# Benjamin-Lee/circkit

Measured on AMD Instinct MI355X. Metric: canonicalize sequences/sec (10M x 1000 b synthetic FASTA payload), higher is better.
Workload: dtype u8

## Files before the change

### circkit_amd/csrc/circkit_hip.hip

```cpp
#include <hip/hip_runtime.h>
#include <stdarg.h>
#include <stdio.h>
#include <stdlib.h>
#include <string.h>
#include <string>
#include <chrono>
#include <vector>

#include "../../include/circkit.h"
#include "canon_core.h"
#include "canon_fast.h"
#include "canon_stream.h"
#include "canon_mixed.h"
#include "fasta_host.h"
#ifndef CK_FAST_WPE
#define CK_FAST_WPE 8
#endif
#ifndef CK_STREAM_WPB
#define CK_STREAM_WPB 16
#endif
#ifndef CK_STREAM_NBUF
#define CK_STREAM_NBUF 2
#endif
#ifndef CK_FAST_BPC
#define CK_FAST_BPC 128
#endif
#include "xxh3_core.h"

namespace {

#ifndef CK_TIER_WPE
#define CK_TIER_WPE 7
#endif
template <int WPB, bool T4 = false>
__global__ __launch_bounds__(WPB * 64, CK_TIER_WPE) void canon_kernel(ck::CanonArgs a, uint32_t nvb, uint32_t* giants)
{
    extern __shared__ __attribute__((aligned(16))) uint32_t lds[];
    uint32_t* blk_count = lds + WPB * a.slice_dw;
    uint32_t* lut = blk_count + 4;
    uint32_t* lutn = lut + ck::FAST_LUT_DW;
    uint32_t live = ~0u;
    if (a.list && gridDim.x < nvb) {
        const uint32_t per = a.segs_per_block, mine = (nvb - blockIdx.x + gridDim.x - 1) / gridDim.x;
        if (threadIdx.x == 0) blk_count[1] = 0;
        __syncthreads();
        uint32_t any = 0;
        for (uint32_t t = threadIdx.x; t < mine * per; t += WPB * 64) {
            const uint32_t j = t / per, sgm = (blockIdx.x + j * gridDim.x) * per + t % per;
            if (sgm < a.in_nseg && a.list_count[sgm]) { any = 1; if (j < 32) atomicOr(blk_count + 1, 1u << j); }
        }
        if (!__syncthreads_or((int)any)) {
            if (a.defer_count)
                for (uint32_t t = threadIdx.x; t < mine; t += WPB * 64) a.defer_count[blockIdx.x + t * gridDim.x] = 0;
            return;
        }
        live = ck::uniform(blk_count[1]);
    }
    ck::fast_lut_init(lut, threadIdx.x, WPB * 64);
    ck::fast_lutn_init(lutn, threadIdx.x, WPB * 64);
    const uint32_t wib = ck::uniform(threadIdx.x >> 6);
    for (uint32_t vb = blockIdx.x, j = 0; vb < nvb; vb += gridDim.x, ++j) {
        if (j < 32 && !((live >> j) & 1u)) {
            if (threadIdx.x == 0 && a.defer_count) a.defer_count[vb] = 0;
            continue;
        }
        if (threadIdx.x == 0) *blk_count = 0;
        __syncthreads();
        ck::canon_wave_loop(a, lds + wib * a.slice_dw, lut, blk_count, vb, nvb, wib, WPB, lutn);
        __syncthreads();
        if (WPB > 1) ck::team_pass(a, lds, lut, lutn, blk_count, vb, wib, WPB, true, T4);
        if (threadIdx.x == 0 && a.defer_count) a.defer_count[vb] = *blk_count;
        if (threadIdx.x == 0 && giants && *blk_count) atomicAdd(giants, *blk_count);
    }
}

constexpr int TEAM_WAVES = 16;
__device__ __forceinline__ void team_stage_block(const ck::CanonArgs& a, uint32_t* buf, uint32_t total_dw, const uint32_t* lut, const uint32_t* lutn,
                                                 uint32_t* blk_count, uint32_t block, uint32_t wib)
{
    ck::CanonArgs solo = a;
    solo.slice_dw = total_dw;
    for (uint32_t sgm = block * a.segs_per_block; sgm < (block + 1) * a.segs_per_block && sgm < a.in_nseg; ++sgm) {
        const uint32_t count = a.list_count[sgm];
        const uint32_t* seg = a.list + (uint64_t)sgm * a.in_seg_cap;
        for (uint32_t i = 0; i < count; ++i) {
            const uint32_t entry = seg[i], rec = entry & ck::ENTRY_REC;
            const uint64_t len = a.offsets[rec + 1] - a.offsets[rec];
            bool done = false, no_2n = (entry & ck::ENTRY_NO_2N) != 0;
            if (len >= 48 && len < (1ull << 31)) {
                const uint32_t n = (uint32_t)len;
                int why = (entry & ck::ENTRY_NOT_ACGT) ? 1 : 3;
                if (why == 3 && ck::need_dw_strand2(n) <= total_dw) { why = ck::canon_record_team2(a, rec, buf, lut, blk_count + 1, wib, TEAM_WAVES); done = why == 0; }
                if (why == 1 && !(entry & ck::ENTRY_NO_2N) && ck::need_dw_2n(n) <= total_dw) {
                    done = ck::canon_record_team2n(a, rec, buf, lut, lutn, blk_count + 1, wib, TEAM_WAVES);
                    no_2n = true;
                }
                if (!done && why == 1 && ck::need_dw_strand4(n) <= total_dw) done = ck::canon_record_team4(a, rec, buf, blk_count + 1, wib, TEAM_WAVES) == 0;
            }
            if (!done) {
                if (wib == 0) {
                    bool not_acgt = (entry & ck::ENTRY_NOT_ACGT) != 0 || no_2n;
                    if (!ck::canon_record(solo, rec, buf, lut, lutn, not_acgt, no_2n)) ck::defer_record(a, blk_count, block, rec, not_acgt, no_2n);
                }
                __syncthreads();
            }
        }
    }
}
__global__ __launch_bounds__(TEAM_WAVES * 64) void canon_team_kernel(ck::CanonArgs a, uint32_t nvb, uint32_t* giants)
{
    extern __shared__ __attribute__((aligned(16))) uint32_t lds[];
    const uint32_t total_dw = TEAM_WAVES * a.slice_dw;
    uint32_t* blk_count = lds + total_dw;
    uint32_t* lut = blk_count + 4;
    uint32_t* lutn = lut + ck::FAST_LUT_DW;
    {
        const uint32_t per = a.segs_per_block, mine = blockIdx.x < nvb ? (nvb - blockIdx.x + gridDim.x - 1) / gridDim.x : 0;
        uint32_t any = 0;
        for (uint32_t t = threadIdx.x; t < mine * per; t += TEAM_WAVES * 64) {
            const uint32_t sgm = (blockIdx.x + (t / per) * gridDim.x) * per + t % per;
            if (sgm < a.in_nseg) any |= a.list_count[sgm];
        }
        if (!__syncthreads_or((int)any)) {
            for (uint32_t t = threadIdx.x; t < mine; t += TEAM_WAVES * 64) a.defer_count[blockIdx.x + t * gridDim.x] = 0;
            return;
        }
    }
    ck::fast_lut_init(lut, threadIdx.x, TEAM_WAVES * 64);
    ck::fast_lutn_init(lutn, threadIdx.x, TEAM_WAVES * 64);
    const uint32_t wib = ck::uniform(threadIdx.x >> 6);
    for (uint32_t vb = blockIdx.x; vb < nvb; vb += gridDim.x) {
        if (threadIdx.x == 0) *blk_count = 0;
        __syncthreads();
        team_stage_block(a, lds, total_dw, lut, lutn, blk_count, vb, wib);
        __syncthreads();
        if (threadIdx.x == 0) {
            a.defer_count[vb] = *blk_count;
            if (giants && *blk_count) atomicAdd(giants, *blk_count);
        }
    }
}

__global__ __launch_bounds__(TEAM_WAVES * 64) void canon_global_kernel(ck::CanonArgs a, ck::CanonArgs a2, uint32_t* scratch, uint32_t* ticket, const uint32_t* giants,
                                                                       const uint32_t* tiers_busy, uint32_t* hint_out)
{
    if (blockIdx.x == 0 && threadIdx.x == 0) *hint_out = *tiers_busy ? 2u : 1u;
    if (*giants == 0) return;
    __shared__ uint32_t blk_count[4], lut[ck::FAST_LUT_DW], lutn[ck::FAST_LUTN_DW], last;
    ck::fast_lut_init(lut, threadIdx.x, TEAM_WAVES * 64);
    ck::fast_lutn_init(lutn, threadIdx.x, TEAM_WAVES * 64);
    const uint32_t wib = ck::uniform(threadIdx.x >> 6);
    if (threadIdx.x == 0) blk_count[0] = 0;
    __syncthreads();
    team_stage_block(a, scratch + (size_t)blockIdx.x * a.slice_dw, a.slice_dw, lut, lutn, blk_count, blockIdx.x, wib);
    __syncthreads();
    if (threadIdx.x == 0) {
        a.defer_count[blockIdx.x] = blk_count[0];
        asm volatile("s_waitcnt vmcnt(0)" ::: "memory");
        __builtin_amdgcn_fence(__ATOMIC_RELEASE, "agent");
        asm volatile("s_waitcnt vmcnt(0)" ::: "memory");
        const uint32_t arrived = atomicAdd(ticket, 1u);
        last = arrived == gridDim.x - 1;
        if (last) {
            __builtin_amdgcn_fence(__ATOMIC_ACQUIRE, "agent");
            asm volatile("s_waitcnt vmcnt(0)" ::: "memory");
            *ticket = 0;
        }
    }
    __syncthreads();
    if (!last) return;
    if (threadIdx.x == 0) blk_count[0] = 0;
    __syncthreads();
    team_stage_block(a2, scratch, a2.slice_dw, lut, lutn, blk_count, 0, wib);
}

__global__ __launch_bounds__(64) void canon_global_one_kernel(ck::CanonArgs a, uint32_t* scratch)
{
    __shared__ uint32_t blk_count, lut[ck::FAST_LUT_DW], lutn[ck::FAST_LUTN_DW];
    ck::fast_lut_init(lut, threadIdx.x, 64);
    ck::fast_lutn_init(lutn, threadIdx.x, 64);
    if (threadIdx.x == 0) blk_count = 0;
    __syncthreads();
    ck::canon_wave_loop(a, scratch, lut, &blk_count, blockIdx.x, gridDim.x, 0, 1, lutn);
}

__global__ __launch_bounds__(64) void xxh3_list_kernel(const uint8_t* bytes, const uint64_t* offsets, const uint32_t* list, uint32_t count,
                                                      uint64_t* out)
{
    for (uint32_t i = blockIdx.x; i < count; i += gridDim.x) {
        const uint32_t r = list[i];
        const uint64_t off = offsets[r];
        const uint64_t h = ck::xxh3_64_wave(bytes + off, (uint32_t)(offsets[r + 1] - off));
        if (ck::lane_id() == 0) out[r] = h;
    }
}

#ifndef CK_STREAM_RPW
#define CK_STREAM_RPW 1
#endif
using StreamC = ck::StreamCfg<CK_STREAM_WPB, CK_STREAM_NBUF, CK_STREAM_RPW, 1>;
#ifndef CK_STREAM_WPB_2
#define CK_STREAM_WPB_2 8
#endif
using StreamC2 = ck::StreamCfg<CK_STREAM_WPB_2, CK_STREAM_NBUF, CK_STREAM_RPW, 2>;
#ifndef CK_STREAM_WPB_HASH
#define CK_STREAM_WPB_HASH 4
#endif
using StreamCH = ck::StreamCfg<CK_STREAM_WPB_HASH, CK_STREAM_NBUF, CK_STREAM_RPW, 1>;
#ifndef CK_STREAM_WPB_ALPHA
#define CK_STREAM_WPB_ALPHA 4
#endif
using StreamCA = ck::StreamCfg<CK_STREAM_WPB_ALPHA, CK_STREAM_NBUF, CK_STREAM_RPW, 1>;
#ifndef CK_STREAM_WPB_PAIR
#define CK_STREAM_WPB_PAIR 8
#endif
#ifndef CK_PAIR_WPE
#define CK_PAIR_WPE 6
#endif
#if CK_STREAM_WPB_PAIR
using StreamCHP = ck::StreamCfg<CK_STREAM_WPB_PAIR, CK_STREAM_NBUF, 2, 1>;
#else
using StreamCHP = StreamCH;
#endif
using StreamCAux = ck::StreamCfg<4, 4, 2, 1>;
using StreamCAux2 = ck::StreamCfg<4, 2, 2, 2>;

__host__ __device__ inline uint32_t count_shift(uint64_t n) { return n <= (1u << 17) ? 0u : (uint32_t)(63 - __builtin_clzll(n)) - 16u; }
__host__ __device__ inline uint64_t count_samples(uint64_t n) { return (n + (1ull << count_shift(n)) - 1) >> count_shift(n); }
__host__ __device__ inline uint32_t stream_mode(uint64_t two, uint64_t lng, uint64_t n)
{
    return lng && lng * 8 >= n ? 3u : (two && two * 4 >= n ? 2u : 1u);
}
constexpr uint32_t CONTENT_SAMPLES = 4096, MODE_ALPHA = 4;
constexpr uint32_t MODE_SHORT = 8, SHORT_MAX_N = 800;
__host__ __device__ inline uint32_t alpha_mode(uint64_t bad, uint64_t sampled) { return bad && bad * 16 >= sampled ? MODE_ALPHA : 0u; }
__host__ __device__ inline uint32_t batch_mode_of(uint64_t two, uint64_t lng, uint64_t n, uint64_t bad, uint64_t sampled, uint64_t shortc, bool hashed)
{
    const uint32_t m = stream_mode(two, lng, n), al = alpha_mode(bad, sampled);
    return (m == 2 && (al || hashed) ? 3u : m) | al | (m == 1 && !al && shortc * 2 >= n ? MODE_SHORT : 0u);
}
__global__ __launch_bounds__(1024) void stream_count_kernel(const uint8_t* __restrict__ bytes, const uint64_t* __restrict__ offsets, uint64_t n, uint32_t* ctl,
                                                            uint32_t* mode, uint32_t* counters, uint32_t hashed)
{
    __shared__ uint32_t blk[4];
    if (threadIdx.x < 4) blk[threadIdx.x] = 0;
    if (blockIdx.x == 0 && threadIdx.x == 3) { counters[0] = 0; counters[1] = 0; counters[3] = 0; counters[16] = 0; counters[17] = 0; }
    __syncthreads();
    const uint32_t shift = count_shift(n);
    const uint64_t ns = count_samples(n);
    uint32_t two = 0, lng = 0, sht = 0;
    for (uint64_t j = (uint64_t)blockIdx.x * 1024 + threadIdx.x; j < ns; j += (uint64_t)gridDim.x * 1024) {
        const uint64_t i = j << shift;
        const uint64_t len = offsets[i + 1] - offsets[i];
        two += len > ck::FAST_MAX_N && len <= ck::FAST2_MAX_N;
        lng += len > ck::FAST2_MAX_N;
        sht += len <= SHORT_MAX_N;
    }
    const uint64_t nc = n < CONTENT_SAMPLES ? n : CONTENT_SAMPLES, cstep = n / nc;
    uint32_t bad = 0;
    for (uint64_t k = (uint64_t)blockIdx.x * 16 + (threadIdx.x >> 6); k < nc; k += (uint64_t)gridDim.x * 16) {
        const uint64_t off = offsets[k * cstep], len = offsets[k * cstep + 1] - off;
        const uint32_t m = len < ck::FAST_MAX_N ? (uint32_t)len : ck::FAST_MAX_N, t = ck::lane_id();
        uint32_t miss = 0;
        if (m >= 16 && 16 * t < m) (void)ck::fast_pack(ck::load16(bytes + off + (16 * t + 16 <= m ? 16 * t : m - 16)), miss);
        bad += ck::ballot(miss != 0) != 0;
    }
    if (ck::ballot(two | lng) != 0) {
        const uint64_t t2 = ck::wave_sum_u64(two), tl = ck::wave_sum_u64(lng);
        if (ck::lane_id() == 0 && t2) atomicAdd(&blk[0], (uint32_t)t2);
        if (ck::lane_id() == 0 && tl) atomicAdd(&blk[1], (uint32_t)tl);
    }
    if (ck::lane_id() == 0 && bad) atomicAdd(&blk[2], bad);
    if (ck::ballot(sht != 0) != 0) {
        const uint64_t ts = ck::wave_sum_u64(sht);
        if (ck::lane_id() == 0) atomicAdd(&blk[3], (uint32_t)ts);
    }
    __syncthreads();
    if (threadIdx.x == 0) {
        if (blk[0]) atomicAdd(ctl, blk[0]);
        if (blk[1]) atomicAdd(ctl + 1, blk[1]);
        if (blk[2]) atomicAdd(ctl + 3, blk[2]);
        if (blk[3]) atomicAdd(ctl + 5, blk[3]);
        asm volatile("s_waitcnt vmcnt(0)" ::: "memory");
        if (atomicAdd(ctl + 2, 1u) == gridDim.x - 1) {
            const uint32_t t2 = atomicExch(ctl, 0u), tl = atomicExch(ctl + 1, 0u), tb = atomicExch(ctl + 3, 0u), ts = atomicExch(ctl + 5, 0u);
            *mode = batch_mode_of(t2, tl, ns, tb, nc, ts, hashed != 0);
            atomicExch(ctl + 2, 0u);
        }
    }
}
__device__ __forceinline__ uint32_t batch_mode(const uint32_t* __restrict__ mode, uint32_t host_mode)
{
    return host_mode ? host_mode & 15u : *mode;
}
template <bool HASH, bool AUX, bool ALPHA>
__global__ __launch_bounds__(256) void canon_rescue_kernel(ck::CanonArgs a, const uint32_t* __restrict__ mode_word, uint32_t host_mode, uint32_t* mode_out,
                                                           uint32_t* tiers_busy)
{
    const uint32_t mode = batch_mode(mode_word, host_mode);
    if (!AUX && ((mode & MODE_ALPHA) != 0) != ALPHA) return;
    if (!AUX && (mode & 3) == 3) return;
    if (blockIdx.x == 0 && threadIdx.x == 0) *mode_out = (host_mode >> 31) ? *mode_word : mode;
    const bool all_records = (mode & 3) == 3;
    if (!all_records) {
        const uint32_t mine = blockIdx.x < a.in_nseg ? (a.in_nseg - blockIdx.x + gridDim.x - 1) / gridDim.x : 0;
        uint32_t any = 0;
        for (uint32_t t = threadIdx.x; t < mine; t += 256) any |= a.list_count[blockIdx.x + t * gridDim.x];
        if (!__syncthreads_or((int)any)) {
            for (uint32_t t = threadIdx.x; t < mine; t += 256) a.defer_count[blockIdx.x + t * gridDim.x] = 0;
            return;
        }
    }
    __shared__ uint32_t lut[ck::FAST_LUT_DW], seg_count;
    ck::fast_lut_init(lut, threadIdx.x, 256);
    ck::RescueState<HASH, AUX> st;
    if (HASH) st.hc = ck::fast_hash_const();
    const uint32_t wib = ck::uniform(threadIdx.x >> 6);
    uint32_t passed_on = 0, walked = 0;
    for (uint32_t sgm = blockIdx.x; sgm < a.in_nseg; sgm += gridDim.x) {
        if (threadIdx.x == 0) seg_count = 0;
        __syncthreads();
        ck::canon_rescue_segment<HASH, AUX, ALPHA>(a, lut, st, &seg_count, sgm, wib, 4, all_records);
        __syncthreads();
        if (threadIdx.x == 0) { a.defer_count[sgm] = seg_count; passed_on += seg_count; ++walked; }
    }
    if (threadIdx.x == 0 && passed_on > walked) *tiers_busy = 1;
}

#ifdef CK_MIXED_TIMELINE
__device__ uint64_t g_timeline[3 * 65536];
#endif
#ifndef CK_MIXED_WPB_PURE
#define CK_MIXED_WPB_PURE 8
#endif
#ifndef CK_MIXED_WPB_HASH
#define CK_MIXED_WPB_HASH 2
#endif
#ifndef CK_MIXED_WPB_N
#define CK_MIXED_WPB_N 4
#endif
constexpr int mixed_wpb(bool nm, bool hash) { return nm ? CK_MIXED_WPB_N : (hash ? CK_MIXED_WPB_HASH : CK_MIXED_WPB_PURE); }
template <bool NM, bool HASH>
__device__ __forceinline__ void canon_mixed_body(const ck::CanonArgs& a, const uint32_t* __restrict__ mode_word, uint32_t host_mode, uint32_t* mode_out, uint32_t* tiers_busy,
                                                 uint32_t* ticket)
{
    constexpr int WPB = mixed_wpb(NM, HASH);
    const uint32_t mode = batch_mode(mode_word, host_mode);
    if ((mode & 3) != 3 || ((mode & MODE_ALPHA) != 0) != NM) return;
    if (blockIdx.x == 0 && threadIdx.x == 0) *mode_out = (host_mode >> 31) ? *mode_word : mode;
#ifdef CK_MIXED_TIMELINE
    const uint64_t tl_start = wall_clock64();
#endif
    extern __shared__ __attribute__((aligned(16))) uint32_t lds[];
    uint32_t* blk_count = lds + WPB * a.slice_dw;
    uint32_t* lut = blk_count + 4;
    uint32_t* lutn = lut + ck::FAST_LUT_DW;
    uint32_t* htab = lutn + ck::LEAN_LUTN_DW;
    ck::fast_lut_init(lut, threadIdx.x, 64 * WPB);
    if (NM) ck::lean_lutn_init(lutn, threadIdx.x, 64 * WPB);
    if (HASH) ck::lean_hash_table_init(htab, threadIdx.x);
    ck::RescueState<HASH, false> st;
    if (HASH) {
        st.hc.k0 = ck::xsec64(8 * (ck::lane_id() >> 2) + 16 * (ck::lane_id() & 3));
        st.hc.k1 = ck::xsec64(8 * (ck::lane_id() >> 2) + 16 * (ck::lane_id() & 3) + 8);
    }
    const uint32_t wib = ck::uniform(threadIdx.x >> 6);
    uint32_t* slice = lds + wib * a.slice_dw;
    const uint64_t payload_end = a.offsets[a.n_records];
    uint32_t passed_on = 0, walked = 0, static_sgm = blockIdx.x;
    for (;;) {
        if (threadIdx.x == 0) { blk_count[0] = 0; blk_count[1] = ticket ? atomicAdd(ticket, 1u) : static_sgm; }
        static_sgm += gridDim.x;
        __syncthreads();
        const uint32_t sgm = blk_count[1];
        if (sgm >= a.in_nseg) break;
        ck::canon_mixed_segment<NM, HASH>(a, slice, lut, st, blk_count, sgm, wib, WPB, payload_end, htab, lutn);
        __syncthreads();
        if (threadIdx.x == 0) { a.defer_count[sgm] = *blk_count; passed_on += *blk_count; ++walked; }
    }
    if (threadIdx.x == 0) {
        if (passed_on > walked) *tiers_busy = 1;
        if (ticket && atomicAdd(ticket + 1, 1u) == gridDim.x - 1) { atomicExch(ticket, 0u); atomicExch(ticket + 1, 0u); }
    }
#ifdef CK_MIXED_TIMELINE
    if (threadIdx.x == 0 && blockIdx.x < 65536) {
        uint32_t hwid;
        asm volatile("s_getreg_b32 %0, hwreg(HW_REG_HW_ID)" : "=s"(hwid));
        uint32_t xcc;
        asm volatile("s_getreg_b32 %0, hwreg(HW_REG_XCC_ID)" : "=s"(xcc));
        g_timeline[3 * blockIdx.x] = tl_start; g_timeline[3 * blockIdx.x + 1] = wall_clock64();
        g_timeline[3 * blockIdx.x + 2] = ((uint64_t)xcc << 32) | hwid;
    }
#endif
}
#ifndef CK_MIXED_NM_VGPR
#define CK_MIXED_NM_VGPR 48
#endif
#ifndef CK_MIXED_H_VGPR
#define CK_MIXED_H_VGPR 40
#endif
#ifndef CK_MIXED_N_SLICE
#define CK_MIXED_N_SLICE 1904
#endif
#ifdef CK_MIXED_WAVES
#define CK_MIXED_ATTR(VGPR, NM, HASH) __launch_bounds__(64 * mixed_wpb(NM, HASH), CK_MIXED_WAVES)
#else
#define CK_MIXED_ATTR(VGPR, NM, HASH) __launch_bounds__(64 * mixed_wpb(NM, HASH)) __attribute__((amdgpu_num_vgpr(VGPR)))
#endif
#define CK_MIXED_KERNEL(NAME, NM, HASH, VGPR)                                                                                                  \
    __global__ CK_MIXED_ATTR(VGPR, NM, HASH) void NAME(ck::CanonArgs a, const uint32_t* __restrict__ mode_word,   \
                                                                                     uint32_t host_mode, uint32_t* mode_out, uint32_t* tiers_busy, uint32_t* ticket) \
    {                                                                                                                                          \
        canon_mixed_body<NM, HASH>(a, mode_word, host_mode, mode_out, tiers_busy, ticket);                                                     \
    }
CK_MIXED_KERNEL(canon_mixed_kernel, false, false, 36)
CK_MIXED_KERNEL(canon_mixed_n_kernel, true, false, CK_MIXED_NM_VGPR)
CK_MIXED_KERNEL(canon_mixed_h_kernel, false, true, CK_MIXED_H_VGPR)
CK_MIXED_KERNEL(canon_mixed_nh_kernel, true, true, CK_MIXED_NM_VGPR)
#undef CK_MIXED_KERNEL

#ifndef CK_GROUP_HASH
#define CK_GROUP_HASH 1
#endif
template <class StreamC, bool HASH, bool AUX, bool PERSIST, bool ALPHA = false>
__global__ __launch_bounds__(StreamC::WPB * 64, (HASH && !AUX && StreamC::ROWS == 1 && (ALPHA || StreamC::RPW == 2)) ? CK_PAIR_WPE : (StreamC::WPB >= 8 || (ALPHA && !HASH && !AUX)) ? CK_FAST_WPE : 4) void canon_stream_kernel(ck::CanonArgs a, const uint32_t* __restrict__ mode,
                                                                                                             uint32_t host_mode, uint32_t nvb)
{
    const uint32_t bm = batch_mode(mode, host_mode);
    if ((bm & 3) != (uint32_t)StreamC::ROWS) return;
    constexpr bool HAS_ALPHA_TWIN = StreamC::ROWS == 1 && !AUX;
    if (HAS_ALPHA_TWIN && ((bm & MODE_ALPHA) != 0) != ALPHA) return;
    if (HAS_ALPHA_TWIN && !ALPHA && !HASH && ((bm & MODE_SHORT) != 0) != (StreamC::RPW == 2)) return;
    constexpr bool GH = CK_GROUP_HASH && HASH && !AUX && StreamC::ROWS == 1 && (StreamC::RPW == 1 || !ALPHA) && StreamC::GROUP <= 16;
    constexpr bool PAIR = GH && StreamC::RPW == 2;
    constexpr bool PAIR_B = !HASH && !AUX && !ALPHA && StreamC::ROWS == 1 && StreamC::RPW == 2;
    __shared__ __attribute__((aligned(16))) uint32_t lds[StreamC::LDS_DW + (GH ? ck::gh_lds_dw<(int)StreamC::GROUP, PAIR>() : PAIR_B ? StreamC::GROUP * ck::PAIR_SCRATCH_DW : 0)];
    uint32_t* lut = lds + StreamC::NBUF * StreamC::BUF_DW;
    uint32_t* blk_count = lut + ck::FAST_LUT_DW;
    uint32_t* gh = lds + StreamC::LDS_DW;
    ck::fast_lut_init(lut, threadIdx.x, StreamC::WPB * 64);
    if (GH) ck::group_hash_init(gh + 2 * StreamC::GROUP * ck::GH_STRIDE_DW, threadIdx.x);
    if (PAIR) ck::group_hash_secret_init(gh + 2 * StreamC::GROUP * ck::GH_STRIDE_DW + ck::GH_CONST_DW, threadIdx.x);
    if (!PERSIST) {
        if (threadIdx.x == 0) *blk_count = 0;
        __syncthreads();
        ck::canon_stream_wave_loop<StreamC, HASH, AUX, GH, ALPHA>(a, lut, lds, blk_count, blockIdx.x, gridDim.x, gh);
        __syncthreads();
        if (threadIdx.x == 0) a.defer_count[blockIdx.x] = *blk_count;
        return;
    }
    for (uint32_t vb = blockIdx.x; vb < nvb; vb += gridDim.x) {
        if (threadIdx.x == 0) *blk_count = 0;
        __syncthreads();
        ck::canon_stream_wave_loop<StreamC, HASH, AUX, GH, ALPHA>(a, lut, lds, blk_count, vb, nvb, gh);
        ck::vmem_wait<0>();
        __syncthreads();
        if (threadIdx.x == 0) a.defer_count[vb] = *blk_count;
    }
}

__global__ __launch_bounds__(256) void xxh3_kernel(const uint8_t* bytes, const uint64_t* offsets, uint64_t n_records,
                                                   uint64_t* out, const uint8_t* hashed, const uint32_t* view, const uint8_t* comp)
{
    const uint32_t wave = ck::uniform(blockIdx.x * 4 + (threadIdx.x >> 6));
    const uint32_t n_waves = gridDim.x * 4;
    const ck::XWaveConst xk = ck::xwave_const();
    __shared__ uint8_t comp_lds[256];
    if (view) { comp_lds[threadIdx.x] = comp[threadIdx.x]; __syncthreads(); comp = comp_lds; }
    if (!hashed) {
        for (uint64_t r = wave; r < n_records; r += n_waves) {
            const uint64_t off = offsets[r];
            const uint64_t h = ck::xxh3_64_wave(bytes + off, (uint32_t)(offsets[r + 1] - off), xk);
            if (ck::lane_id() == 0) out[r] = h;
        }
        return;
    }
    const uint64_t per_wave = (n_records + n_waves - 1) / n_waves;
    const uint32_t span = per_wave >= 512 ? 512u : (per_wave <= 64 ? 64u : (uint32_t)((per_wave + 63) / 64) * 64u);
    for (uint64_t big = (uint64_t)wave * span; big < n_records; big += (uint64_t)n_waves * span) {
      const uint64_t f0 = big + 8 * ck::lane_id();
      uint64_t flags8 = ~0ull;
      if (f0 < n_records && 8 * ck::lane_id() < span) {
          flags8 = *reinterpret_cast<const uint64_t*>(hashed + f0);
          if (n_records - f0 < 8) flags8 |= ~0ull << (8 * (n_records - f0));
      }
      if (ck::ballot(((flags8 - 0x0101010101010101ull) & ~flags8 & 0x8080808080808080ull) != 0) == 0) continue;
      for (uint64_t base = big; base < big + span && base < n_records; base += 64) {
        const uint64_t mine = base + ck::lane_id();
        const bool need = mine < n_records && !hashed[mine];
        uint64_t todo = ck::ballot(need);
        if (!todo) continue;
        const uint64_t my_off = need ? offsets[mine] : 0;
        const uint32_t my_len = need ? (uint32_t)(offsets[mine + 1] - my_off) : 0u;
        const bool mine_short = need && my_len <= 240u;
        const uint64_t shorts = ck::ballot(mine_short);
        if (shorts) {
            if (mine_short) {
                const uint8_t* p = bytes + my_off;
                uint64_t h;
                if (view) {
                    const uint32_t v = view[mine], rot = v & 0x7FFFFFFFu;
                    h = ck::xxh3_short(ck::XView{ p, my_len, rot < my_len ? rot : 0u, (v >> 31) != 0, comp }, my_len);
                } else h = ck::xxh3_short(ck::XPlain{ p }, my_len);
                out[mine] = h;
            }
            todo &= ~shorts;
        }
        while (todo) {
            const uint32_t l = (uint32_t)ck::ffs64(todo);
            todo &= todo - 1;
            const uint64_t off = ((uint64_t)ck::readlane((uint32_t)(my_off >> 32), l) << 32) | ck::readlane((uint32_t)my_off, l);
            const uint32_t len = ck::readlane(my_len, l);
            const uint64_t h = view ? ck::xxh3_64_wave_view(bytes + off, len, view[base + l], comp, xk) : ck::xxh3_64_wave(bytes + off, len, xk);
            if (ck::lane_id() == 0) out[base + l] = h;
        }
      }
    }
}

__device__ __forceinline__ uint64_t splitmix64(uint64_t x)
{
    x += 0x9E3779B97F4A7C15ULL;
    x = (x ^ (x >> 30)) * 0xBF58476D1CE4E5B9ULL;
    x = (x ^ (x >> 27)) * 0x94D049BB133111EBULL;
    return x ^ (x >> 31);
}

__global__ __launch_bounds__(256) void synth_fill_kernel(uint64_t seed, uint64_t first_base, uint64_t n_bases,
                                                         uint8_t* out)
{
    const uint64_t key = seed * 0xD1342543DE82EF95ULL;
    const uint64_t stride = (uint64_t)gridDim.x * blockDim.x * 16;
    for (uint64_t i = ((uint64_t)blockIdx.x * blockDim.x + threadIdx.x) * 16; i < n_bases; i += stride) {
        const uint64_t g0 = first_base + i;
        uint64_t wi = g0 >> 5, w = splitmix64(key + wi);
        uint32_t o[4] = { 0, 0, 0, 0 };
#pragma unroll
        for (int b = 0; b < 16; ++b) {
            const uint64_t g = g0 + b;
            if ((g >> 5) != wi) { wi = g >> 5; w = splitmix64(key + wi); }
            const uint32_t code = (uint32_t)(w >> (2 * (g & 31))) & 3u;
            o[b >> 2] |= ((0x54474341u >> (8 * code)) & 0xFFu) << (8 * (b & 3));
        }
        if (i + 16 <= n_bases) {
            ck::store16(out + i, ck::u32x4{ o[0], o[1], o[2], o[3] });
        } else {
            for (uint64_t b = 0; i + b < n_bases; ++b) out[i + b] = (uint8_t)(o[b >> 2] >> (8 * (b & 3)));
        }
    }
}

typedef uint32_t copy_v4 __attribute__((ext_vector_type(4)));
template <int UNROLL>
__global__ __launch_bounds__(256) void bench_copy_kernel(const copy_v4* __restrict__ in, copy_v4* __restrict__ out, uint64_t n16)
{
    const uint64_t stride = (uint64_t)gridDim.x * 256 * UNROLL;
    uint64_t i = (uint64_t)blockIdx.x * 256 * UNROLL + threadIdx.x;
    for (; i + 256 * (UNROLL - 1) < n16; i += stride) {
        copy_v4 r[UNROLL];
#pragma unroll
        for (int u = 0; u < UNROLL; ++u) r[u] = in[i + u * 256];
#pragma unroll
        for (int u = 0; u < UNROLL; ++u) out[i + u * 256] = r[u];
    }
    for (; i < n16; i += 256) out[i] = in[i];
}

__global__ void fixed_offsets_kernel(uint64_t base, uint64_t len, uint64_t n, uint64_t* off)
{
    const uint64_t stride = (uint64_t)gridDim.x * blockDim.x;
    for (uint64_t i = (uint64_t)blockIdx.x * blockDim.x + threadIdx.x; i <= n; i += stride) off[i] = base + i * len;
}

constexpr uint64_t UNIQ_EMPTY = ~0ull;
struct __attribute__((aligned(16))) UniqSlot { unsigned long long key, val; };
__device__ __forceinline__ uint64_t uniq_slot(uint64_t h, uint64_t mask) { return (h ^ (h >> 29)) & mask; }
__device__ __forceinline__ UniqSlot uniq_peek(const UniqSlot* p)
{
    typedef unsigned long long v2 __attribute__((ext_vector_type(2)));
    const v2 v = *reinterpret_cast<const v2*>(p);
    return UniqSlot{ v.x, v.y };
}
__device__ __forceinline__ bool uniq_fold(UniqSlot* t, uint64_t mask, uint64_t h, unsigned long long v)
{
    if (h == UNIQ_EMPTY) { atomicMin(&t[mask + 1].val, v); return true; }
    uint64_t s = uniq_slot(h, mask), probes = 0;
    for (;;) {
        const UniqSlot cur = uniq_peek(t + s);
        if (cur.key == h) {
            if (cur.val > v) atomicMin(&t[s].val, v);
            return true;
        }
        if (cur.key == UNIQ_EMPTY) {
            const unsigned long long old = atomicCAS(&t[s].key, (unsigned long long)UNIQ_EMPTY, (unsigned long long)h);
            if (old == UNIQ_EMPTY || old == h) { atomicMin(&t[s].val, v); return true; }
        }
        s = (s + 1) & mask;
        if (++probes > mask) return false;
    }
}

__global__ __launch_bounds__(256) void uniq_insert_kernel(const uint64_t* __restrict__ hash, const uint64_t* __restrict__ index, uint64_t n, uint64_t base,
                                                          UniqSlot* t, uint64_t mask, uint32_t* status)
{
    const uint64_t stride = (uint64_t)gridDim.x * blockDim.x;
    for (uint64_t i = (uint64_t)blockIdx.x * blockDim.x + threadIdx.x; i < n; i += stride)
        if (!uniq_fold(t, mask, hash[i], index ? index[i] : base + i)) atomicAdd(status, 1u);
}

__global__ __launch_bounds__(256) void uniq_lookup_kernel(const uint64_t* __restrict__ hash, uint64_t n, const UniqSlot* __restrict__ t, uint64_t mask,
                                                          uint64_t* first_seen, uint8_t* keep, uint64_t base)
{
    const uint64_t stride = (uint64_t)gridDim.x * blockDim.x;
    for (uint64_t i = (uint64_t)blockIdx.x * blockDim.x + threadIdx.x; i < n; i += stride) {
        const uint64_t h = hash[i];
        uint64_t r = UNIQ_EMPTY;
        if (h == UNIQ_EMPTY) {
            r = t[mask + 1].val;
        } else {
            uint64_t s = uniq_slot(h, mask), probes = 0;
            for (;;) {
                const UniqSlot cur = uniq_peek(t + s);
                if (cur.key == h) { r = cur.val; break; }
                if (cur.key == UNIQ_EMPTY || ++probes > mask) break;
                s = (s + 1) & mask;
            }
        }
        first_seen[i] = r;
        if (keep) keep[i] = r == base + i;
    }
}

__device__ __forceinline__ bool uniq_fold_local(UniqSlot* t, uint64_t mask, uint64_t h, uint32_t i)
{
    if (h == UNIQ_EMPTY) { atomicMin(reinterpret_cast<unsigned int*>(&t[mask + 1].val), i); return true; }
    uint64_t s = uniq_slot(h, mask), probes = 0;
    for (;;) {
        const UniqSlot cur = uniq_peek(t + s);
        unsigned int* halves = reinterpret_cast<unsigned int*>(&t[s].val);
        if (cur.key == h) {
            const uint32_t lo = (uint32_t)cur.val, hi = (uint32_t)(cur.val >> 32);
            if ((lo < hi ? lo : hi) > i) atomicMin(halves, i);
            return true;
        }
        if (cur.key == UNIQ_EMPTY) {
            const unsigned long long old = atomicCAS(&t[s].key, (unsigned long long)UNIQ_EMPTY, (unsigned long long)h);
            if (old == UNIQ_EMPTY) { halves[1] = i; return true; }
            if (old == h) { atomicMin(halves, i); return true; }
        }
        s = (s + 1) & mask;
        if (++probes > mask) return false;
    }
}
__global__ __launch_bounds__(256) void uniq_resolve_insert_kernel(const uint64_t* __restrict__ hash, uint64_t n, UniqSlot* t, uint64_t mask, uint32_t* status,
                                                                  const uint32_t* only_if = nullptr)
{
    if (only_if && *only_if == 0) return;
    const uint64_t stride = (uint64_t)gridDim.x * blockDim.x;
    for (uint64_t i = (uint64_t)blockIdx.x * blockDim.x + threadIdx.x; i < n; i += stride)
        if (!uniq_fold_local(t, mask, hash[i], (uint32_t)i)) atomicAdd(status, 1u);
}
__global__ __launch_bounds__(256) void uniq_resolve_lookup_kernel(const uint64_t* __restrict__ hash, uint64_t n, const UniqSlot* __restrict__ t, uint64_t mask,
                                                                  uint64_t* first_seen, uint8_t* keep, uint64_t base, const uint32_t* only_if = nullptr)
{
    if (only_if && *only_if == 0) return;
    const uint64_t stride = (uint64_t)gridDim.x * blockDim.x;
    for (uint64_t i = (uint64_t)blockIdx.x * blockDim.x + threadIdx.x; i < n; i += stride) {
        const uint64_t h = hash[i];
        uint64_t v = UNIQ_EMPTY;
        if (h == UNIQ_EMPTY) {
            v = t[mask + 1].val;
        } else {
            uint64_t s = uniq_slot(h, mask), probes = 0;
            for (;;) {
                const UniqSlot cur = uniq_peek(t + s);
                if (cur.key == h) { v = cur.val; break; }
                if (cur.key == UNIQ_EMPTY || ++probes > mask) break;
                s = (s + 1) & mask;
            }
        }
        const uint32_t lo = (uint32_t)v, hi = (uint32_t)(v >> 32), r = lo < hi ? lo : hi;
        first_seen[i] = r == 0xFFFFFFFFu ? UNIQ_EMPTY : base + r;
        if (keep) keep[i] = r == (uint32_t)i;
    }
}

__global__ __launch_bounds__(256) void uniq_rehash_kernel(const UniqSlot* __restrict__ old, uint64_t oslots, UniqSlot* t, uint64_t mask)
{
    const uint64_t stride = (uint64_t)gridDim.x * blockDim.x;
    for (uint64_t i = (uint64_t)blockIdx.x * blockDim.x + threadIdx.x; i < oslots; i += stride) {
        const UniqSlot e = uniq_peek(old + i);
        if (i + 1 == oslots) { if (e.val != UNIQ_EMPTY) atomicMin(&t[mask + 1].val, e.val); continue; }
        if (e.key != UNIQ_EMPTY) (void)uniq_fold(t, mask, e.key, e.val);
    }
}

constexpr uint32_t UNIQ_MAX_WORLD = 64;
__device__ __forceinline__ uint32_t uniq_owner(uint64_t h, uint32_t world) { return (uint32_t)((h >> 20) & 0x7FFFFFFFu) % world; }
__global__ __launch_bounds__(256) void uniq_partition_count_kernel(const uint64_t* __restrict__ hash, uint64_t n, uint32_t world, unsigned long long* counts)
{
    __shared__ uint32_t hist[UNIQ_MAX_WORLD];
    if (threadIdx.x < UNIQ_MAX_WORLD) hist[threadIdx.x] = 0;
    __syncthreads();
    const uint64_t stride = (uint64_t)gridDim.x * blockDim.x;
    for (uint64_t i = (uint64_t)blockIdx.x * blockDim.x + threadIdx.x; i < n; i += stride) atomicAdd(&hist[uniq_owner(hash[i], world)], 1u);
    __syncthreads();
    if (threadIdx.x < world && hist[threadIdx.x]) atomicAdd(&counts[threadIdx.x], (unsigned long long)hist[threadIdx.x]);
}
__global__ __launch_bounds__(256) void uniq_partition_scatter_kernel(const uint64_t* __restrict__ hash, uint64_t n, uint64_t base, uint32_t world,
                                                                     const unsigned long long* __restrict__ counts, unsigned long long* cursor,
                                                                     uint64_t* rows, uint32_t* slot)
{
    __shared__ uint32_t hist[UNIQ_MAX_WORLD];
    __shared__ unsigned long long first[UNIQ_MAX_WORLD], start[UNIQ_MAX_WORLD];
    constexpr uint32_t PER = 4;
    const uint64_t chunk = 256ull * PER;
    if (threadIdx.x < UNIQ_MAX_WORLD) {
        unsigned long long v = threadIdx.x < world ? counts[threadIdx.x] : 0ull, incl = v;
        for (uint32_t d = 1; d < UNIQ_MAX_WORLD; d <<= 1) {
            const uint32_t lo = ck::shfl((uint32_t)incl, threadIdx.x - d), hi = ck::shfl((uint32_t)(incl >> 32), threadIdx.x - d);
            if (threadIdx.x >= d) incl += ((unsigned long long)hi << 32) | lo;
        }
        first[threadIdx.x] = incl - v;
    }
    for (uint64_t c0 = (uint64_t)blockIdx.x * chunk; c0 < n; c0 += (uint64_t)gridDim.x * chunk) {
        if (threadIdx.x < UNIQ_MAX_WORLD) hist[threadIdx.x] = 0;
        __syncthreads();
        uint32_t rank[PER];
#pragma unroll
        for (uint32_t k = 0; k < PER; ++k) {
            const uint64_t i = c0 + k * 256 + threadIdx.x;
            rank[k] = i < n ? atomicAdd(&hist[uniq_owner(hash[i], world)], 1u) : 0u;
        }
        __syncthreads();
        if (threadIdx.x < world)
            start[threadIdx.x] = first[threadIdx.x] + (hist[threadIdx.x] ? atomicAdd(&cursor[threadIdx.x], (unsigned long long)hist[threadIdx.x]) : 0ull);
        __syncthreads();
#pragma unroll
        for (uint32_t k = 0; k < PER; ++k) {
            const uint64_t i = c0 + k * 256 + threadIdx.x;
            if (i < n) {
                const uint64_t h = hash[i];
                const uint64_t pos = start[uniq_owner(h, world)] + rank[k];
                typedef unsigned long long v2 __attribute__((ext_vector_type(2)));
                *reinterpret_cast<v2*>(rows + 2 * pos) = v2{ h, base + i };
                slot[i] = (uint32_t)pos;
            }
        }
        __syncthreads();
    }
}
__global__ __launch_bounds__(256) void uniq_insert_rows_kernel(const uint64_t* __restrict__ rows, uint64_t n, UniqSlot* t, uint64_t mask, uint32_t* status)
{
    const uint64_t stride = (uint64_t)gridDim.x * blockDim.x;
    for (uint64_t i = (uint64_t)blockIdx.x * blockDim.x + threadIdx.x; i < n; i += stride) {
        const UniqSlot r = uniq_peek(reinterpret_cast<const UniqSlot*>(rows) + i);
        if (!uniq_fold(t, mask, r.key, r.val)) atomicAdd(status, 1u);
    }
}
__global__ __launch_bounds__(256) void uniq_lookup_rows_kernel(const uint64_t* __restrict__ rows, uint64_t n, const UniqSlot* __restrict__ t, uint64_t mask,
                                                               uint64_t* answers)
{
    const uint64_t stride = (uint64_t)gridDim.x * blockDim.x;
    for (uint64_t i = (uint64_t)blockIdx.x * blockDim.x + threadIdx.x; i < n; i += stride) {
        const uint64_t h = rows[2 * i];
        uint64_t r = UNIQ_EMPTY;
        if (h == UNIQ_EMPTY) {
            r = t[mask + 1].val;
        } else {
            uint64_t s = uniq_slot(h, mask), probes = 0;
            for (;;) {
                const UniqSlot cur = uniq_peek(t + s);
                if (cur.key == h) { r = cur.val; break; }
                if (cur.key == UNIQ_EMPTY || ++probes > mask) break;
                s = (s + 1) & mask;
            }
        }
        answers[i] = r;
    }
}
__global__ __launch_bounds__(256) void uniq_gather_kernel(const uint64_t* __restrict__ answers, const uint32_t* __restrict__ slot, uint64_t n, uint64_t base,
                                                          uint64_t* first_seen, uint8_t* keep)
{
    const uint64_t stride = (uint64_t)gridDim.x * blockDim.x;
    for (uint64_t i = (uint64_t)blockIdx.x * blockDim.x + threadIdx.x; i < n; i += stride) {
        const uint64_t r = answers[slot[i]];
        first_seen[i] = r;
        if (keep) keep[i] = r == base + i;
    }
}

__global__ __launch_bounds__(256) void uniq_clear_kernel(UniqSlot* t, uint64_t slots, uint32_t* overflow, const uint32_t* only_if = nullptr)
{
    if (only_if && *only_if == 0) return;
    typedef unsigned long long v2 __attribute__((ext_vector_type(2)));
    if (overflow && blockIdx.x == 0 && threadIdx.x == 0) *overflow = 0;
    const uint64_t stride = (uint64_t)gridDim.x * blockDim.x;
    for (uint64_t i = (uint64_t)blockIdx.x * blockDim.x + threadIdx.x; i < slots; i += stride)
        *reinterpret_cast<v2*>(t + i) = v2{ UNIQ_EMPTY, UNIQ_EMPTY };
}

#ifndef CK_BKT_NW
#define CK_BKT_NW 512
#endif
constexpr uint32_t BKT_NW = CK_BKT_NW, BKT_SLOTS = 4096, BKT_MAX = 3072, BKT_KEYS = 2600, BKT_MAX_LOG2 = 13;
__device__ __forceinline__ uint32_t bkt_of(uint64_t h, uint32_t log2b) { return (uint32_t)(h >> (64 - log2b)); }
__global__ __launch_bounds__(1024) void uniq_bkt_count_kernel(const uint64_t* __restrict__ hash, uint64_t n, uint64_t per, uint32_t log2b, uint32_t* counts,
                                                              uint32_t* flag, uint32_t* overflow)
{
    extern __shared__ uint32_t bkt_lds[];
    const uint32_t B = 1u << log2b;
    for (uint32_t b = threadIdx.x; b < B; b += 1024) bkt_lds[b] = 0;
    if (blockIdx.x == 0 && threadIdx.x == 0) { *flag = 0; *overflow = 0; }
    __syncthreads();
    const uint64_t i0 = (uint64_t)blockIdx.x * per, i1 = i0 + per < n ? i0 + per : n;
    for (uint64_t i = i0 + threadIdx.x; i < i1; i += 1024) atomicAdd(&bkt_lds[bkt_of(hash[i], log2b)], 1u);
    __syncthreads();
    for (uint32_t b = threadIdx.x; b < B; b += 1024) counts[(uint64_t)blockIdx.x * B + b] = bkt_lds[b];
}
__global__ __launch_bounds__(1024) void uniq_bkt_colscan_kernel(uint32_t* counts, uint32_t B, uint32_t* tot)
{
    __shared__ uint32_t seg[16][64];
    constexpr uint32_t PER = BKT_NW / 16;
    const uint32_t bl = threadIdx.x & 63, sg = threadIdx.x >> 6, b = blockIdx.x * 64 + bl;
    uint32_t sum = 0;
    for (uint32_t w = sg * PER; w < (sg + 1) * PER; ++w) sum += counts[(uint64_t)w * B + b];
    seg[sg][bl] = sum;
    __syncthreads();
    uint32_t run = 0;
    for (uint32_t k = 0; k < sg; ++k) run += seg[k][bl];
    for (uint32_t w = sg * PER; w < (sg + 1) * PER; ++w) {
        const uint64_t k = (uint64_t)w * B + b;
        const uint32_t cnt = counts[k];
        counts[k] = run;
        run += cnt;
    }
    if (sg == 15) tot[b] = run;
}
__global__ __launch_bounds__(1024) void uniq_bkt_basescan_kernel(const uint32_t* __restrict__ tot, uint32_t B, uint32_t* base)
{
    __shared__ uint32_t part[1024];
    const uint32_t items = (B + 1023) / 1024, b0 = threadIdx.x * items;
    uint32_t sum = 0;
    for (uint32_t k = 0; k < items; ++k) if (b0 + k < B) sum += tot[b0 + k];
    part[threadIdx.x] = sum;
    __syncthreads();
    for (uint32_t d = 1; d < 1024; d <<= 1) {
        const uint32_t v = threadIdx.x >= d ? part[threadIdx.x - d] : 0u;
        __syncthreads();
        part[threadIdx.x] += v;
        __syncthreads();
    }
    uint32_t run = part[threadIdx.x] - sum;
    for (uint32_t k = 0; k < items; ++k) if (b0 + k < B) { base[b0 + k] = run; run += tot[b0 + k]; }
    if (threadIdx.x == 1023) base[B] = part[1023];
}
__global__ __launch_bounds__(1024) void uniq_bkt_scatter_kernel(const uint64_t* __restrict__ hash, uint64_t n, uint64_t per, uint32_t log2b,
                                                                const uint32_t* __restrict__ counts, const uint32_t* __restrict__ base, uint64_t* rows,
                                                                uint64_t* first_seen, uint64_t base_index)
{
    extern __shared__ uint32_t bkt_lds[];
    const uint32_t B = 1u << log2b;
    for (uint32_t b = threadIdx.x; b < B; b += 1024) bkt_lds[b] = base[b] + counts[(uint64_t)blockIdx.x * B + b];
    __syncthreads();
    const uint64_t i0 = (uint64_t)blockIdx.x * per, i1 = i0 + per < n ? i0 + per : n;
    typedef unsigned long long v2 __attribute__((ext_vector_type(2)));
    constexpr int U = 4;
    uint64_t i = i0 + threadIdx.x;
    for (; i + (U - 1) * 1024 < i1; i += U * 1024) {
        uint64_t h[U];
#pragma unroll
        for (int u = 0; u < U; ++u) h[u] = hash[i + u * 1024];
#pragma unroll
        for (int u = 0; u < U; ++u) {
            const uint32_t pos = atomicAdd(&bkt_lds[bkt_of(h[u], log2b)], 1u);
            *reinterpret_cast<v2*>(rows + 2 * (uint64_t)pos) = v2{ h[u], i + u * 1024 };
            first_seen[i + u * 1024] = base_index + i + u * 1024;
        }
    }
    for (; i < i1; i += 1024) {
        const uint64_t h = hash[i];
        const uint32_t pos = atomicAdd(&bkt_lds[bkt_of(h, log2b)], 1u);
        *reinterpret_cast<v2*>(rows + 2 * (uint64_t)pos) = v2{ h, i };
        first_seen[i] = base_index + i;
    }
}
#ifndef BKT_RESOLVE_T
#define BKT_RESOLVE_T 1024
#endif
__global__ __launch_bounds__(BKT_RESOLVE_T) void uniq_bkt_resolve_kernel(const uint64_t* __restrict__ rows, const uint32_t* __restrict__ base, uint64_t base_index,
                                                               uint64_t* first_seen, uint8_t* keep, uint32_t* flag)
{
    __shared__ unsigned long long keys[BKT_SLOTS];
    __shared__ uint32_t idx[BKT_SLOTS], special;
    const uint32_t r0 = base[blockIdx.x], cnt = base[blockIdx.x + 1] - r0;
    if (cnt == 0) return;
    if (cnt > BKT_MAX) { if (threadIdx.x == 0) atomicExch(flag, 1u); return; }
    for (uint32_t s = threadIdx.x; s < BKT_SLOTS; s += BKT_RESOLVE_T) { keys[s] = UNIQ_EMPTY; idx[s] = 0xFFFFFFFFu; }
    if (threadIdx.x == 0) special = 0xFFFFFFFFu;
    __syncthreads();
    constexpr uint32_t RPT = (BKT_MAX + BKT_RESOLVE_T - 1) / BKT_RESOLVE_T;
    uint64_t hk[RPT];
    uint32_t ik[RPT];
#pragma unroll
    for (uint32_t k = 0; k < RPT; ++k) {
        const uint32_t r = threadIdx.x + k * BKT_RESOLVE_T;
        hk[k] = 0; ik[k] = 0xFFFFFFFFu;
        if (r < cnt) { const UniqSlot row = uniq_peek(reinterpret_cast<const UniqSlot*>(rows) + r0 + r); hk[k] = row.key; ik[k] = (uint32_t)row.val; }
    }
#pragma unroll
    for (uint32_t k = 0; k < RPT; ++k) {
        if (ik[k] == 0xFFFFFFFFu) continue;
        const uint64_t h = hk[k];
        if (h == UNIQ_EMPTY) { atomicMin(&special, ik[k]); continue; }
        uint32_t s = (uint32_t)(h ^ (h >> 29)) & (BKT_SLOTS - 1);
        for (;;) {
            const unsigned long long old = atomicCAS(&keys[s], (unsigned long long)UNIQ_EMPTY, (unsigned long long)h);
            if (old == UNIQ_EMPTY || old == h) { atomicMin(&idx[s], ik[k]); break; }
            s = (s + 1) & (BKT_SLOTS - 1);
        }
    }
    __syncthreads();
#pragma unroll
    for (uint32_t k = 0; k < RPT; ++k) {
        if (ik[k] == 0xFFFFFFFFu) continue;
        const uint64_t h = hk[k];
        uint32_t m;
        if (h == UNIQ_EMPTY) m = special;
        else {
            uint32_t s = (uint32_t)(h ^ (h >> 29)) & (BKT_SLOTS - 1);
            while (keys[s] != h) s = (s + 1) & (BKT_SLOTS - 1);
            m = idx[s];
        }
        if (m != ik[k]) first_seen[ik[k]] = base_index + m;
    }
}
__global__ __launch_bounds__(256) void uniq_keep_kernel(const uint64_t* __restrict__ first_seen, uint64_t n, uint64_t base, uint8_t* keep, const uint32_t* skip_if)
{
    if (skip_if && *skip_if != 0) return;
    const uint64_t stride = (uint64_t)gridDim.x * blockDim.x;
    for (uint64_t i = (uint64_t)blockIdx.x * blockDim.x + threadIdx.x; i < n; i += stride) keep[i] = first_seen[i] == base + i;
}

#ifndef CK_RESCUE_BPC
#define CK_RESCUE_BPC 8
#endif
#ifndef CK_TIER_BPC
#define CK_TIER_BPC 128
#endif
#ifndef CK_TIER_BPC_IDLE
#define CK_TIER_BPC_IDLE 8
#endif
#ifndef CK_TIER_A
#define CK_TIER_A 1280
#endif
#ifndef CK_TIER_B1
#define CK_TIER_B1 1900
#endif
#ifndef CK_TIER_B2
#define CK_TIER_B2 3324
#endif
constexpr int N_TIERS = 5;
constexpr uint32_t TIER_DW[N_TIERS] = { CK_TIER_A, CK_TIER_B1, CK_TIER_B2, 9980, CK_LUT_STRIDE == 1 ? 40188u : 31996u };
constexpr uint32_t TIER_EXTRA_DW = 4 + ck::FAST_LUT_DW + ck::FAST_LUTN_DW;
constexpr uint32_t TIER_D_DW = TIER_DW[N_TIERS - 1];
constexpr int BATCH_TIERS = 3;
constexpr uint32_t BATCH_SLICE_DW[BATCH_TIERS - 1] = { CK_TIER_A, 9980 / 4 };
constexpr uint32_t TEAM_SLICE_DW = TIER_D_DW / 16;
constexpr int N_CU = 256;

}

struct circkit_ctx {
    int device = -1;
    hipStream_t own_stream = nullptr, stream = nullptr;
    hipEvent_t ev0 = nullptr, ev1 = nullptr;
    hipEvent_t ev_order = nullptr;
    static constexpr int MAX_PARTS = 32;
    hipStream_t s_in = nullptr, s_out = nullptr;
    hipEvent_t ev_in[MAX_PARTS] = {}, ev_done[MAX_PARTS] = {}, ev_head = nullptr;
    bool timed = false;
    std::string err;
    uint8_t* d_comp = nullptr;
    uint32_t* d_counters = nullptr;
    uint32_t* d_lists[N_TIERS + 1] = {};
    uint32_t* d_seg_counts = nullptr;
    uint64_t list_cap = 0, seg_alloc = 0;
    uint8_t *d_in = nullptr, *d_out = nullptr, *d_strand = nullptr;
    uint64_t* d_off = nullptr; uint32_t* d_idx = nullptr; uint64_t* d_hash = nullptr;
    uint64_t cap_bytes = 0, cap_rec = 0;
    uint32_t* d_view = nullptr; uint64_t cap_view = 0;
    uint8_t* d_hashed = nullptr; uint64_t cap_hashed = 0;
    uint32_t* d_gscratch = nullptr; uint64_t cap_gscratch = 0;
    uint64_t gscratch_default = 256ull << 20;
    uint64_t* h_off = nullptr;
    uint64_t h_off_cap = 0;
    volatile uint32_t* h_mode = nullptr;
    uint32_t* d_mode = nullptr;
    UniqSlot* d_table = nullptr;
    uint64_t uniq_mask = 0, uniq_count = 0;
    uint32_t mode_seen = 0;
    bool uniq_local = false;
    bool uniq_lost = false;

    void* orfs = nullptr;
    void (*orfs_release)(void*) = nullptr;
    void* monomerize = nullptr;
    void (*monomerize_release)(void*) = nullptr;
};

hipStream_t ck_ctx_stream(circkit_ctx* c) { return c->stream; }
int ck_ctx_device(circkit_ctx* c) { return c->device; }
int ck_ctx_fail(circkit_ctx* c, int code, const char* msg) { c->err = msg; return code; }
void** ck_ctx_orfs_slot(circkit_ctx* c, void (*release)(void*)) { c->orfs_release = release; return &c->orfs; }
void** ck_ctx_monomerize_slot(circkit_ctx* c, void (*release)(void*)) { c->monomerize_release = release; return &c->monomerize; }

namespace {

int fail(circkit_ctx* c, int code, const char* fmt, ...)
{
    char buf[512];
    va_list ap; va_start(ap, fmt); vsnprintf(buf, sizeof buf, fmt, ap); va_end(ap);
    if (c) c->err = buf;
    return code;
}

#define CK_HIP(c, call)                                                                             \
    do {                                                                                            \
        hipError_t e_ = (call);                                                                     \
        if (e_ != hipSuccess)                                                                       \
            return fail(c, e_ == hipErrorOutOfMemory ? CIRCKIT_ERR_OOM : CIRCKIT_ERR_HIP,           \
                        "%s failed: %s", #call, hipGetErrorString(e_));                             \
    } while (0)

int ensure_lists(circkit_ctx* c, uint64_t entries, uint64_t segs)
{
    if (entries > c->list_cap) {
        c->list_cap = 0;
        for (int i = 0; i < N_TIERS + 1; ++i) {
            if (c->d_lists[i]) { (void)hipFree(c->d_lists[i]); c->d_lists[i] = nullptr; }
            CK_HIP(c, hipMalloc(&c->d_lists[i], entries * sizeof(uint32_t)));
        }
        c->list_cap = entries;
    }
    if (segs > c->seg_alloc) {
        if (c->d_seg_counts) { (void)hipFree(c->d_seg_counts); c->d_seg_counts = nullptr; }
        c->seg_alloc = 0;
        CK_HIP(c, hipMalloc(&c->d_seg_counts, (N_TIERS + 1) * segs * sizeof(uint32_t)));
        c->seg_alloc = segs;
    }
    return CIRCKIT_OK;
}

int ensure_gscratch(circkit_ctx* c, uint64_t bytes)
{
    if (bytes <= c->cap_gscratch) return CIRCKIT_OK;
    if (c->d_gscratch) { (void)hipFree(c->d_gscratch); c->d_gscratch = nullptr; c->cap_gscratch = 0; }
    CK_HIP(c, hipMalloc(&c->d_gscratch, bytes));
    c->cap_gscratch = bytes;
    return CIRCKIT_OK;
}

inline uint64_t worst_case_dw(uint64_t n) { return 2 * ((n + 3) / 4 + 2) + (n + 31) / 32 + 1 + 64; }
constexpr uint64_t GSLICE1_DW = 1ull << 20;

int launch_canon(circkit_ctx* c, const uint8_t* d_bytes, const uint64_t* d_offsets, uint64_t n, uint8_t* d_out,
                 uint32_t* d_idx, uint8_t* d_strand, uint64_t* d_hash, uint32_t flags, uint32_t host_mode = 0, bool keep_status = false)
{
#ifdef CK_FORCE_HOST_MODE
    if (!host_mode) host_mode = CK_FORCE_HOST_MODE;
#endif
    if (n >= (1ull << 30)) return fail(c, CIRCKIT_ERR_INVALID_ARG, "n_records must be < 2^30");
    CK_HIP(c, hipSetDevice(c->device));
    if (n == 0) { c->timed = false; return CIRCKIT_OK; }
    const bool device_decides = host_mode == 0;
    uint32_t guess_flag = 0;
    if (device_decides) {
        static const bool no_guess = getenv("CIRCKIT_NO_MODE_GUESS") != nullptr;
        const uint32_t seen = *c->h_mode & 15u;
        if (!no_guess && (seen & 3u) && seen == c->mode_seen) { host_mode = seen; guess_flag = 0x80000000u; }
        c->mode_seen = seen;
        static const bool dbg = getenv("CIRCKIT_DEBUG_MODE_GUESS") != nullptr;
        if (dbg) fprintf(stderr, "[mode guess] n=%llu report=%u -> %s\n", (unsigned long long)n, seen, guess_flag ? "guessed" : "decided on the device");
    }
    const uint32_t kmode = host_mode | guess_flag;
    const bool aux = d_idx || d_strand || (flags & ck::CK_FLAG_FWD_ONLY);
    const uint64_t per_step = aux ? StreamCAux::GROUP : StreamC::GROUP;
    const uint64_t blocks = (n + per_step - 1) / per_step;
    unsigned G = (unsigned)(blocks < (uint64_t)N_CU * CK_FAST_BPC ? blocks : (uint64_t)N_CU * CK_FAST_BPC);
    const unsigned G_small = (unsigned)(n < (uint64_t)N_CU * 16 ? n : (uint64_t)N_CU * 16);
    if (G < G_small) G = G_small;
    uint32_t cap = (uint32_t)(per_step * ((blocks + G - 1) / G));
    uint32_t all_cap = (uint32_t)((n + G - 1) / G);
    uint32_t taper_seg0 = 0, taper_log2 = 0;
#ifndef CK_NO_TAPER
#ifndef CK_TAPER_DIV
#define CK_TAPER_DIV 16
#endif
    if (G >= 4096 && all_cap >= (2u << CK_TAPER_GENS)) {
        while ((2u << taper_log2) <= G / CK_TAPER_DIV) ++taper_log2;
        const uint64_t gen = 1ull << taper_log2;
        taper_seg0 = G - (uint32_t)(CK_TAPER_GENS * gen);
        auto tapered = [&](uint32_t A) { uint64_t t = 0; for (int j = 1; j <= CK_TAPER_GENS; ++j) t += A >> j; return t; };
        while ((uint64_t)taper_seg0 * all_cap + gen * tapered(all_cap) < n) ++all_cap;
        if (cap < all_cap) cap = all_cap;
    }
#endif
    int rc = ensure_lists(c, (uint64_t)G * cap + 1024ull * cap, G < 256u ? 256u : G);
    if (rc) return rc;
    if (!c->d_gscratch && (rc = ensure_gscratch(c, c->gscratch_default))) return rc;
    uint32_t* view = nullptr;
    if (d_hash && !d_out) {
        if (n > c->cap_view) {
            if (c->d_view) { (void)hipFree(c->d_view); c->d_view = nullptr; c->cap_view = 0; }
            CK_HIP(c, hipMalloc(&c->d_view, (n + n / 8 + 64) * sizeof(uint32_t)));
            c->cap_view = n + n / 8 + 64;
        }
        view = c->d_view;
    }
    if (d_hash) {
        if (n > c->cap_hashed) {
            if (c->d_hashed) { (void)hipFree(c->d_hashed); c->d_hashed = nullptr; c->cap_hashed = 0; }
            CK_HIP(c, hipMalloc(&c->d_hashed, n + n / 8 + 64));
            c->cap_hashed = n + n / 8 + 64;
        }
        CK_HIP(c, hipMemsetAsync(c->d_hashed, 0, n, c->stream));
    }
    if (!device_decides) CK_HIP(c, hipMemsetAsync(c->d_counters, 0, (keep_status ? 3 : 4) * sizeof(uint32_t), c->stream));
    CK_HIP(c, hipEventRecord(c->ev0, c->stream));
    ck::CanonArgs a{};
    a.bytes = d_bytes; a.offsets = d_offsets; a.n_records = n;
    a.out_bytes = d_out; a.out_index = d_idx; a.out_strand = d_strand; a.out_hash = d_hash; a.hashed = c->d_hashed; a.out_view = view;
    a.comp_lut = c->d_comp; a.status = c->d_counters + 3; a.flags = flags;
    a.list = nullptr; a.list_count = nullptr; a.all_seg_cap = all_cap; a.taper_seg0 = taper_seg0; a.taper_log2 = taper_log2;
    a.defer_list = c->d_lists[0]; a.defer_count = c->d_seg_counts; a.out_seg_cap = cap;
    a.slice_dw = 0;
    const uint32_t* counts = c->d_counters + 5;
    {
        if (device_decides) {
            const uint64_t ns = count_samples(n);
            const unsigned cgrid = (unsigned)((ns + 1023) / 1024 < 128 ? (ns + 1023) / 1024 : 128);
            hipLaunchKernelGGL(stream_count_kernel, dim3(cgrid), dim3(1024), 0, c->stream, d_bytes, d_offsets, n, c->d_counters + 8, c->d_counters + 5, c->d_counters, (d_hash && !aux) ? 1u : 0u);
        }
        const uint32_t seen = *c->h_mode;
        const uint32_t expect = host_mode ? host_mode & 3 : ((seen & 3) ? seen & 3 : 1u);
        const unsigned small = G < 2u * N_CU ? G : 2u * N_CU;
        const dim3 block(StreamC::WPB * 64), block_aux(StreamCAux::WPB * 64), block_h(StreamCH::WPB * 64), block_hp(StreamCHP::WPB * 64), block_a(StreamCA::WPB * 64), block_2(StreamC2::WPB * 64);
        const uint32_t expect_alpha = host_mode ? host_mode & MODE_ALPHA : seen & MODE_ALPHA;
        for (uint32_t rows = 1; rows <= 2; ++rows) {
            if (host_mode && (host_mode & 3) != rows) continue;
            for (uint32_t alpha = 0; alpha <= (rows == 1 && !aux ? 1u : 0u); ++alpha) {
                if (host_mode && rows == 1 && !aux && ((host_mode & MODE_ALPHA) != 0) != (alpha != 0)) continue;
                const bool full = expect == rows && (rows != 1 || aux || (expect_alpha != 0) == (alpha != 0));
                const dim3 grid(full ? G : small);
#define CK_LAUNCH_STREAM(CFG, H, A, BLK, AL)                                                                                         \
                do {                                                                                                                \
                    if (full) hipLaunchKernelGGL((canon_stream_kernel<CFG, H, A, false, AL>), grid, BLK, 0, c->stream, a, counts, kmode, G); \
                    else hipLaunchKernelGGL((canon_stream_kernel<CFG, H, A, true, AL>), grid, BLK, 0, c->stream, a, counts, kmode, G);       \
                } while (0)
                if (rows == 1) {
                    if (aux) CK_LAUNCH_STREAM(StreamCAux, true, true, block_aux, false);
                    else if (d_hash) { if (alpha) CK_LAUNCH_STREAM(StreamCH, true, false, block_h, true); else CK_LAUNCH_STREAM(StreamCHP, true, false, block_hp, false); }
                    else if (alpha) CK_LAUNCH_STREAM(StreamCA, false, false, block_a, true);
                    else {
                        const bool expect_short = ((host_mode ? host_mode : seen) & MODE_SHORT) != 0;
                        for (int sh = 0; sh < 2; ++sh) {
                            if (host_mode && (sh != 0) != expect_short) continue;
                            const bool full_sh = full && (sh != 0) == expect_short;
                            const dim3 grid_sh(full_sh ? G : small);
                            if (sh) { if (full_sh) hipLaunchKernelGGL((canon_stream_kernel<StreamCHP, false, false, false, false>), grid_sh, block_hp, 0, c->stream, a, counts, kmode, G);
                                      else hipLaunchKernelGGL((canon_stream_kernel<StreamCHP, false, false, true, false>), grid_sh, block_hp, 0, c->stream, a, counts, kmode, G); }
                            else { if (full_sh) hipLaunchKernelGGL((canon_stream_kernel<StreamC, false, false, false, false>), grid_sh, block, 0, c->stream, a, counts, kmode, G);
                                   else hipLaunchKernelGGL((canon_stream_kernel<StreamC, false, false, true, false>), grid_sh, block, 0, c->stream, a, counts, kmode, G); }
                        }
                    }
                } else {
                    if (aux) CK_LAUNCH_STREAM(StreamCAux2, true, true, block_aux, false);
                    else if (d_hash) CK_LAUNCH_STREAM(StreamC2, true, false, block_2, false);
                    else CK_LAUNCH_STREAM(StreamC2, false, false, block_2, false);
                }
#undef CK_LAUNCH_STREAM
            }
        }
    }
    unsigned nseg = G;
    uint32_t seg_cap = cap;
    {
        const unsigned grid = nseg < (unsigned)N_CU * CK_RESCUE_BPC ? nseg : (unsigned)N_CU * CK_RESCUE_BPC;
        a.list = c->d_lists[0]; a.list_count = c->d_seg_counts;
        a.in_nseg = nseg; a.in_seg_cap = seg_cap; a.segs_per_block = 1;
        a.defer_list = c->d_lists[1]; a.defer_count = c->d_seg_counts + c->seg_alloc; a.out_seg_cap = seg_cap;
#ifdef CK_NO_PINNED_MODE
        uint32_t* mode_out = c->d_counters + 6;
#else
        uint32_t* mode_out = c->d_mode;
#endif
        const bool mixed_has_it = host_mode && !aux && (host_mode & 3) == 3;
        const bool lean = (!host_mode || !(host_mode & MODE_ALPHA)) && !mixed_has_it, alpha = (!host_mode || (host_mode & MODE_ALPHA)) && !mixed_has_it;
        if (aux) hipLaunchKernelGGL((canon_rescue_kernel<true, true, false>), dim3(grid), dim3(256), 0, c->stream, a, counts, kmode, mode_out, c->d_counters + 1);
        else if (d_hash) {
            if (lean) hipLaunchKernelGGL((canon_rescue_kernel<true, false, false>), dim3(grid), dim3(256), 0, c->stream, a, counts, kmode, mode_out, c->d_counters + 1);
            if (alpha) hipLaunchKernelGGL((canon_rescue_kernel<true, false, true>), dim3(grid), dim3(256), 0, c->stream, a, counts, kmode, mode_out, c->d_counters + 1);
        } else {
            if (lean) hipLaunchKernelGGL((canon_rescue_kernel<false, false, false>), dim3(grid), dim3(256), 0, c->stream, a, counts, kmode, mode_out, c->d_counters + 1);
            if (alpha) hipLaunchKernelGGL((canon_rescue_kernel<false, false, true>), dim3(grid), dim3(256), 0, c->stream, a, counts, kmode, mode_out, c->d_counters + 1);
        }
    }
    if (!aux && (!host_mode || (host_mode & 3) == 3)) {
        const uint32_t seen = *c->h_mode;
        const unsigned walking = nseg < (unsigned)N_CU * CK_RESCUE_BPC ? nseg : (unsigned)N_CU * CK_RESCUE_BPC;
#ifdef CK_NO_PINNED_MODE
        uint32_t* mode_out = c->d_counters + 6;
#else
        uint32_t* mode_out = c->d_mode;
#endif
        for (uint32_t nm = 0; nm < 2; ++nm) {
            if (host_mode && ((host_mode & MODE_ALPHA) != 0) != (nm != 0)) continue;
            const bool expected = host_mode ? true : ((seen & 3) == 3 && ((seen & MODE_ALPHA) != 0) == (nm != 0));
            const unsigned resident = (unsigned)N_CU * (20u / (unsigned)mixed_wpb(true, false));
#ifdef CK_MIXED_N_STATIC
            const unsigned full = nseg;
#else
            const unsigned full = nm ? (nseg < resident ? nseg : resident) : nseg;
#endif
            const unsigned grid = expected ? full : walking;
#ifdef CK_MIXED_N_STATIC
            uint32_t* ticket = nullptr;
#else
            uint32_t* ticket = nm ? c->d_counters + 16 : nullptr;
#endif
            a.slice_dw = nm ? CK_MIXED_N_SLICE : TIER_DW[0];
            const int mwpb = nm ? mixed_wpb(true, d_hash != nullptr) : (d_hash ? mixed_wpb(false, true) : mixed_wpb(false, false));
            const size_t shmem = ((size_t)mwpb * a.slice_dw + 4 + ck::FAST_LUT_DW + ck::LEAN_LUTN_DW + (d_hash ? ck::LEAN_HASH_TABLE_DW : 0)) * 4;
            if (d_hash) {
                if (nm) hipLaunchKernelGGL(canon_mixed_nh_kernel, dim3(grid), dim3(64 * mwpb), shmem, c->stream, a, counts, kmode, mode_out, c->d_counters + 1, ticket);
                else hipLaunchKernelGGL(canon_mixed_h_kernel, dim3(grid), dim3(64 * mwpb), shmem, c->stream, a, counts, kmode, mode_out, c->d_counters + 1, ticket);
            } else {
                if (nm) hipLaunchKernelGGL(canon_mixed_n_kernel, dim3(grid), dim3(64 * mwpb), shmem, c->stream, a, counts, kmode, mode_out, c->d_counters + 1, ticket);
                else hipLaunchKernelGGL(canon_mixed_kernel, dim3(grid), dim3(64 * mwpb), shmem, c->stream, a, counts, kmode, mode_out, c->d_counters + 1, ticket);
            }
        }
    }
#ifdef CK_DEBUG_DUMP
    {
        (void)hipStreamSynchronize(c->stream);
        std::vector<uint32_t> cnt(nseg);
        (void)hipMemcpy(cnt.data(), c->d_seg_counts + c->seg_alloc, nseg * 4, hipMemcpyDeviceToHost);
        uint64_t total = 0; unsigned shown = 0;
        if (getenv("CK_DUMP_HIST")) {
            std::vector<uint32_t> ents((size_t)nseg * seg_cap);
            (void)hipMemcpy(ents.data(), c->d_lists[1], ents.size() * 4, hipMemcpyDeviceToHost);
            std::vector<uint64_t> offs(n + 1);
            (void)hipMemcpy(offs.data(), d_offsets, (n + 1) * 8, hipMemcpyDeviceToHost);
            uint64_t hist[2][32] = {}, bytes[2] = {};
            for (unsigned sg = 0; sg < nseg; ++sg)
                for (uint32_t k = 0; k < cnt[sg]; ++k) {
                    const uint32_t e = ents[(size_t)sg * seg_cap + k]; const uint64_t len = offs[(e & ck::ENTRY_REC) + 1] - offs[e & ck::ENTRY_REC];
                    hist[e >> 31][63 - __builtin_clzll(len | 1)]++; bytes[e >> 31] += len;
                }
            for (int f = 0; f < 2; ++f) { fprintf(stderr, "[dump] flag %d (%llu bytes):", f, (unsigned long long)bytes[f]); for (int b = 0; b < 32; ++b) if (hist[f][b]) fprintf(stderr, " 2^%d:%llu", b, (unsigned long long)hist[f][b]); fprintf(stderr, "\n"); }
        }
        for (unsigned sg = 0; sg < nseg; ++sg) {
            total += cnt[sg];
            for (uint32_t k = 0; k < cnt[sg] && shown < 12; ++k, ++shown) {
                uint32_t e = 0; uint64_t o[2];
                (void)hipMemcpy(&e, c->d_lists[1] + (uint64_t)sg * seg_cap + k, 4, hipMemcpyDeviceToHost);
                (void)hipMemcpy(o, d_offsets + (e & ck::ENTRY_REC), 16, hipMemcpyDeviceToHost);
                fprintf(stderr, "[dump] seg %u entry %u: rec %u flag %u len %llu\n", sg, k, e & ck::ENTRY_REC, e >> 31, (unsigned long long)(o[1] - o[0]));
            }
        }
        fprintf(stderr, "[dump] stage A input: %llu records in %u segments\n", (unsigned long long)total, nseg);
    }
#endif
    const bool tiers_idle = c->h_mode[1] == 1;
    for (int t = 0; t < BATCH_TIERS; ++t) {
        const bool last = t == BATCH_TIERS - 1;
        const unsigned spb = t == 0 ? 1 : (last ? (nseg + N_CU - 1) / N_CU : (nseg >= 16u * N_CU ? 4 : 1));
        const unsigned grid = (nseg + spb - 1) / spb;
        a.list = c->d_lists[t + 1]; a.list_count = c->d_seg_counts + (uint64_t)(t + 1) * c->seg_alloc;
        a.in_nseg = nseg; a.in_seg_cap = seg_cap; a.segs_per_block = spb;
        a.defer_list = last ? c->d_lists[0] : c->d_lists[t + 2];
        a.defer_count = last ? c->d_seg_counts : c->d_seg_counts + (uint64_t)(t + 2) * c->seg_alloc;
        a.out_seg_cap = spb * seg_cap;
        a.slice_dw = last ? TEAM_SLICE_DW : BATCH_SLICE_DW[t];
        const unsigned bpc = tiers_idle ? CK_TIER_BPC_IDLE : CK_TIER_BPC;
        const unsigned launched = grid < (unsigned)N_CU * bpc ? grid : (unsigned)N_CU * bpc;
        if (last) hipLaunchKernelGGL(canon_team_kernel, dim3(launched), dim3(TEAM_WAVES * 64), (TEAM_WAVES * TEAM_SLICE_DW + TIER_EXTRA_DW) * 4, c->stream, a, grid, c->d_counters);
        else if (tiers_idle) hipLaunchKernelGGL((canon_kernel<4, false>), dim3(launched), dim3(256), (4 * a.slice_dw + TIER_EXTRA_DW) * 4, c->stream, a, grid, (uint32_t*)nullptr);
        else hipLaunchKernelGGL((canon_kernel<4, true>), dim3(launched), dim3(256), (4 * a.slice_dw + TIER_EXTRA_DW) * 4, c->stream, a, grid, (uint32_t*)nullptr);
        nseg = grid;
        seg_cap = spb * seg_cap;
    }
    {
        const uint64_t cap_dw = c->cap_gscratch / 4;
        const uint64_t slice1 = cap_dw < GSLICE1_DW ? cap_dw : GSLICE1_DW;
        const unsigned max_w1 = (unsigned)(cap_dw / slice1 < 64 ? cap_dw / slice1 : 64);
        const unsigned spb1 = (nseg + max_w1 - 1) / max_w1, w1 = (nseg + spb1 - 1) / spb1;
        a.list = c->d_lists[0]; a.list_count = c->d_seg_counts;
        a.in_nseg = nseg; a.in_seg_cap = seg_cap; a.segs_per_block = spb1;
        a.defer_list = c->d_lists[1]; a.defer_count = c->d_seg_counts + c->seg_alloc; a.out_seg_cap = spb1 * seg_cap;
        a.slice_dw = (uint32_t)slice1;
        ck::CanonArgs a2 = a;
        a2.list = c->d_lists[1]; a2.list_count = c->d_seg_counts + c->seg_alloc;
        a2.in_nseg = w1; a2.in_seg_cap = spb1 * seg_cap; a2.segs_per_block = w1;
        a2.defer_list = nullptr; a2.defer_count = nullptr; a2.out_seg_cap = 0;
        a2.slice_dw = (uint32_t)(cap_dw < 0xFFFFFFFFull ? cap_dw : 0xFFFFFFFFull);
        hipLaunchKernelGGL(canon_global_kernel, dim3(w1), dim3(TEAM_WAVES * 64), 0, c->stream, a, a2, c->d_gscratch, c->d_counters + 2, (const uint32_t*)c->d_counters,
                           (const uint32_t*)(c->d_counters + 1), c->d_mode + 1);
    }
    if (d_hash) {
        if (view) hipLaunchKernelGGL(xxh3_kernel, dim3(G < 2048u ? G : 2048u), dim3(256), 0, c->stream, d_bytes, d_offsets, n, d_hash, (const uint8_t*)c->d_hashed,
                                     (const uint32_t*)view, (const uint8_t*)c->d_comp);
        else hipLaunchKernelGGL(xxh3_kernel, dim3(G < 2048u ? G : 2048u), dim3(256), 0, c->stream, d_out, d_offsets, n, d_hash, (const uint8_t*)c->d_hashed,
                                (const uint32_t*)nullptr, (const uint8_t*)nullptr);
    }
    CK_HIP(c, hipEventRecord(c->ev1, c->stream));
    CK_HIP(c, hipGetLastError());
    c->timed = true;
    return CIRCKIT_OK;
}

int launch_single(circkit_ctx* c, const uint8_t* d_bytes, const uint64_t* d_offsets, uint64_t len, uint8_t* d_out, uint32_t* d_idx,
                  uint8_t* d_strand, uint64_t* d_hash, uint32_t flags)
{
    ck::CanonArgs a{};
    a.bytes = d_bytes; a.offsets = d_offsets; a.n_records = 1;
    a.out_bytes = d_out; a.out_index = d_idx; a.out_strand = d_strand; a.out_hash = nullptr; a.hashed = nullptr;
    a.comp_lut = c->d_comp; a.status = c->d_counters + 3; a.flags = flags;
    CK_HIP(c, hipMemsetAsync(c->d_counters + 3, 0, sizeof(uint32_t), c->stream));
    const uint64_t need = worst_case_dw(len);
    int t = 0;
    while (t < N_TIERS && TIER_DW[t] < need) ++t;
    if (t < N_TIERS) {
        a.slice_dw = TIER_DW[t];
        hipLaunchKernelGGL(canon_kernel<1>, dim3(1), dim3(64), (TIER_DW[t] + TIER_EXTRA_DW) * 4, c->stream, a, 1u, (uint32_t*)nullptr);
    } else {
        int rc = ensure_gscratch(c, need * 4);
        if (rc) return rc;
        a.slice_dw = (uint32_t)(need < 0xFFFFFFFFull ? need : 0xFFFFFFFFull);
        hipLaunchKernelGGL(canon_global_one_kernel, dim3(1), dim3(64), 0, c->stream, a, c->d_gscratch);
    }
    if (d_hash) hipLaunchKernelGGL(xxh3_kernel, dim3(1), dim3(256), 0, c->stream, d_out, d_offsets, (uint64_t)1, d_hash, (const uint8_t*)nullptr, (const uint32_t*)nullptr, (const uint8_t*)nullptr);
    CK_HIP(c, hipGetLastError());
    c->timed = false;
    return CIRCKIT_OK;
}

template <class T>
int grow(circkit_ctx* c, T*& p, uint64_t want_elems)
{
    if (p) { (void)hipFree(p); p = nullptr; }
    CK_HIP(c, hipMalloc(&p, want_elems * sizeof(T)));
    return CIRCKIT_OK;
}

int ensure_staging(circkit_ctx* c, uint64_t bytes, uint64_t recs)
{
    if (bytes + 64 > c->cap_bytes) {
        const uint64_t nb = bytes + bytes / 8 + 4096;
        c->cap_bytes = 0;
        int rc;
        if ((rc = grow(c, c->d_in, nb))) return rc;
        if ((rc = grow(c, c->d_out, nb))) return rc;
        c->cap_bytes = nb;
    }
    if (recs + 1 > c->cap_rec) {
        const uint64_t nr = recs + recs / 8 + 1024;
        c->cap_rec = 0;
        int rc;
        if ((rc = grow(c, c->d_off, nr))) return rc;
        if ((rc = grow(c, c->d_idx, nr))) return rc;
        if ((rc = grow(c, c->d_strand, nr))) return rc;
        if ((rc = grow(c, c->d_hash, nr))) return rc;
        c->cap_rec = nr;
    }
    return CIRCKIT_OK;
}

int host_batch_enqueue(circkit_ctx* c, const uint8_t* bytes, const uint64_t* offsets, uint64_t n, uint8_t* out,
                       uint32_t* idx, uint8_t* strand, uint64_t* hash, uint32_t flags);
int host_batch(circkit_ctx* c, const uint8_t* bytes, const uint64_t* offsets, uint64_t n, uint8_t* out,
               uint32_t* idx, uint8_t* strand, uint64_t* hash, uint32_t flags)
{
    if (!c) return CIRCKIT_ERR_INVALID_ARG;
    const int rc = host_batch_enqueue(c, bytes, offsets, n, out, idx, strand, hash, flags);
    if (rc != CIRCKIT_OK) {
        if (c->s_in) (void)hipStreamSynchronize(c->s_in);
        if (c->stream) (void)hipStreamSynchronize(c->stream);
        if (c->s_out) (void)hipStreamSynchronize(c->s_out);
    }
    return rc;
}
int host_batch_enqueue(circkit_ctx* c, const uint8_t* bytes, const uint64_t* offsets, uint64_t n, uint8_t* out,
                       uint32_t* idx, uint8_t* strand, uint64_t* hash, uint32_t flags)
{
    if (n && (!offsets || offsets[0] != 0)) return fail(c, CIRCKIT_ERR_INVALID_ARG, "offsets[0] must be 0");
    if (n == 0) return CIRCKIT_OK;
    const uint64_t total = offsets[n];
    if (total && !bytes) return fail(c, CIRCKIT_ERR_INVALID_ARG, "bytes is NULL");
    CK_HIP(c, hipSetDevice(c->device));
    int rc = ensure_staging(c, total, n);
    if (rc) return rc;
    const bool need_bytes = out || hash;
    static const bool dbg_t = getenv("CIRCKIT_DEBUG_TIMING") != nullptr;
    auto dbg_t0 = std::chrono::steady_clock::now();
    auto dbg_lap = [&](const char* what) {
        if (!dbg_t) return;
        const auto now = std::chrono::steady_clock::now();
        fprintf(stderr, "  host_batch %-18s %.3f ms\n", what, std::chrono::duration<double>(now - dbg_t0).count() * 1e3);
        dbg_t0 = now;
    };
    uint64_t two_word = 0, longer = 0, shorter = 0, max_len = 0;
    for (uint64_t i = 0; i < n; ++i) {
        if (offsets[i + 1] < offsets[i]) return fail(c, CIRCKIT_ERR_INVALID_ARG, "offsets decrease at record %llu", (unsigned long long)i);
        const uint64_t len = offsets[i + 1] - offsets[i];
        two_word += len > ck::FAST_MAX_N && len <= ck::FAST2_MAX_N;
        longer += len > ck::FAST2_MAX_N;
        shorter += len <= SHORT_MAX_N;
        max_len = len > max_len ? len : max_len;
    }
    if (max_len >> 31) return fail(c, CIRCKIT_ERR_TOO_LONG, "a record of 2^31 symbols or more (cyclic positions are 32-bit)");
    if (n == 1 && (max_len + 15) / 16 + 2 <= TIER_DW[0]) {
        if (total) CK_HIP(c, hipMemcpyAsync(c->d_in, bytes, total, hipMemcpyHostToDevice, c->stream));
        CK_HIP(c, hipMemcpyAsync(c->d_off, offsets, (n + 1) * 8, hipMemcpyHostToDevice, c->stream));
        rc = launch_single(c, c->d_in, c->d_off, max_len, need_bytes ? c->d_out : nullptr, idx ? c->d_idx : nullptr,
                           strand ? c->d_strand : nullptr, hash ? c->d_hash : nullptr, flags);
        if (rc) return rc;
        if (out && total) CK_HIP(c, hipMemcpyAsync(out, c->d_out, total, hipMemcpyDeviceToHost, c->stream));
        if (idx) CK_HIP(c, hipMemcpyAsync(idx, c->d_idx, n * 4, hipMemcpyDeviceToHost, c->stream));
        if (strand) CK_HIP(c, hipMemcpyAsync(strand, c->d_strand, n, hipMemcpyDeviceToHost, c->stream));
        if (hash) CK_HIP(c, hipMemcpyAsync(hash, c->d_hash, n * 8, hipMemcpyDeviceToHost, c->stream));
        uint32_t unprocessed = 0;
        CK_HIP(c, hipMemcpyAsync(&unprocessed, c->d_counters + 3, 4, hipMemcpyDeviceToHost, c->stream));
        CK_HIP(c, hipStreamSynchronize(c->stream));
        if (unprocessed) return fail(c, CIRCKIT_ERR_TOO_LONG, "%u record(s) could not be processed", unprocessed);
        return CIRCKIT_OK;
    }
    if (worst_case_dw(max_len) > TIER_D_DW && (rc = ensure_gscratch(c, worst_case_dw(max_len) * 4))) return rc;
    dbg_lap("offset scan");
    int parts = (int)(total / (16ull << 20));
    parts = parts < 1 ? 1 : (parts > 8 ? 8 : parts);
    if (total > (512ull << 20)) { parts = (int)(total / (64ull << 20)); parts = parts > 16 ? 16 : parts; }
    parts = parts > circkit_ctx::MAX_PARTS ? circkit_ctx::MAX_PARTS : parts;
    if ((uint64_t)parts > n) parts = (int)n;
    if (getenv("CIRCKIT_HOST_BATCH_PARTS")) { const int p = atoi(getenv("CIRCKIT_HOST_BATCH_PARTS")); if (p >= 1 && p <= circkit_ctx::MAX_PARTS && (uint64_t)p <= n) parts = p; }
    static const bool plain_streams = getenv("CIRCKIT_HOST_BATCH_PLAIN_STREAMS") != nullptr;
    const bool inline_h2d = !plain_streams;
    if (!c->s_out) {
        if (plain_streams) {
            CK_HIP(c, hipStreamCreateWithFlags(&c->s_in, hipStreamNonBlocking));
            CK_HIP(c, hipStreamCreateWithFlags(&c->s_out, hipStreamNonBlocking));
        } else {
            int prio_least = 0, prio_greatest = 0;
            CK_HIP(c, hipDeviceGetStreamPriorityRange(&prio_least, &prio_greatest));
            CK_HIP(c, hipStreamCreateWithPriority(&c->s_out, hipStreamNonBlocking, prio_greatest));
        }
        CK_HIP(c, hipEventCreateWithFlags(&c->ev_head, hipEventDisableTiming));
        for (int k = 0; k < circkit_ctx::MAX_PARTS; ++k) {
            CK_HIP(c, hipEventCreateWithFlags(&c->ev_in[k], hipEventDisableTiming));
            CK_HIP(c, hipEventCreateWithFlags(&c->ev_done[k], hipEventDisableTiming));
        }
    }
    uint64_t cut[circkit_ctx::MAX_PARTS + 1];
    cut[0] = 0; cut[parts] = n;
    for (int k = 1; k < parts; ++k) {
        const uint64_t want = total / parts * k;
        uint64_t lo = cut[k - 1] + 1, hi = n - (parts - k);
        if (lo > hi) lo = hi;
        while (lo < hi) { const uint64_t mid = (lo + hi) / 2; if (offsets[mid] < want) lo = mid + 1; else hi = mid; }
        cut[k] = lo;
    }
    CK_HIP(c, hipEventRecord(c->ev_head, c->stream));
    if (!inline_h2d) CK_HIP(c, hipStreamWaitEvent(c->s_in, c->ev_head, 0));
    if (n + 1 > c->h_off_cap) {
        if (c->h_off) { (void)hipHostFree((void*)c->h_off); c->h_off = nullptr; c->h_off_cap = 0; }
        const uint64_t cap = n + 1 + (n + 1) / 8 + 1024;
        CK_HIP(c, hipHostMalloc((void**)&c->h_off, cap * (8 + 8 + 4 + 1), hipHostMallocDefault));
        c->h_off_cap = cap;
    }
    uint64_t* const st_hash = c->h_off + c->h_off_cap;
    uint32_t* const st_idx = (uint32_t*)(st_hash + c->h_off_cap);
    uint8_t* const st_strand = (uint8_t*)(st_idx + c->h_off_cap);
    memcpy(c->h_off, offsets, (n + 1) * 8);
    hipStream_t sin = inline_h2d ? c->stream : c->s_in;
    CK_HIP(c, hipMemcpyAsync(c->d_off, c->h_off, (n + 1) * 8, hipMemcpyHostToDevice, sin));
    auto copy_in = [&](int k) -> int {
        const uint64_t b0 = offsets[cut[k]], b1 = offsets[cut[k + 1]];
        if (b1 > b0) CK_HIP(c, hipMemcpyAsync(c->d_in + b0, bytes + b0, b1 - b0, hipMemcpyHostToDevice, sin));
        if (!inline_h2d) CK_HIP(c, hipEventRecord(c->ev_in[k], sin));
        return CIRCKIT_OK;
    };
    for (int k = 0; k < (inline_h2d ? 1 : parts); ++k) if ((rc = copy_in(k))) return rc;
    dbg_lap("enqueue copy-in");
    const uint64_t nc = n < CONTENT_SAMPLES / 8 ? n : CONTENT_SAMPLES / 8, cstep = n / nc;
    uint64_t bad = 0;
    {
        static const struct Acgt { uint8_t no[256]; Acgt() { memset(no, 1, sizeof no); no['A'] = no['C'] = no['G'] = no['T'] = 0; } } acgt;
        for (uint64_t k = 0; k < nc; ++k) {
            const uint64_t o = offsets[k * cstep], len = offsets[k * cstep + 1] - o, m = len < ck::FAST_MAX_N ? len : ck::FAST_MAX_N;
            uint32_t b = 0;
            for (uint64_t i = 0; i < m; ++i) b |= acgt.no[bytes[o + i]];
            bad += b;
        }
    }
    const uint32_t host_mode = batch_mode_of(two_word, longer, n, bad, nc, shorter, hash != nullptr && !idx && !strand && !(flags & ck::CK_FLAG_FWD_ONLY));
    dbg_lap("content sample");
    volatile uint32_t* unprocessed = c->h_mode + 4;
    for (int k = 0; k < parts; ++k) {
        const uint64_t r0 = cut[k], nk = cut[k + 1] - r0, b0 = offsets[r0], b1 = offsets[cut[k + 1]];
        if (!inline_h2d) CK_HIP(c, hipStreamWaitEvent(c->stream, c->ev_in[k], 0));
        rc = launch_canon(c, c->d_in, c->d_off + r0, nk, need_bytes ? c->d_out : nullptr, idx ? c->d_idx + r0 : nullptr,
                          strand ? c->d_strand + r0 : nullptr, hash ? c->d_hash + r0 : nullptr, flags, host_mode, k > 0);
        if (rc) return rc;
        CK_HIP(c, hipEventRecord(c->ev_done[k], c->stream));
        CK_HIP(c, hipStreamWaitEvent(c->s_out, c->ev_done[k], 0));
        if (inline_h2d && k + 1 < parts && (rc = copy_in(k + 1))) return rc;
        if (out && b1 > b0) CK_HIP(c, hipMemcpyAsync(out + b0, c->d_out + b0, b1 - b0, hipMemcpyDeviceToHost, c->s_out));
        if (idx) CK_HIP(c, hipMemcpyAsync(st_idx + r0, c->d_idx + r0, nk * 4, hipMemcpyDeviceToHost, c->s_out));
        if (strand) CK_HIP(c, hipMemcpyAsync(st_strand + r0, c->d_strand + r0, nk, hipMemcpyDeviceToHost, c->s_out));
        if (hash) CK_HIP(c, hipMemcpyAsync(st_hash + r0, c->d_hash + r0, nk * 8, hipMemcpyDeviceToHost, c->s_out));
    }
    unprocessed[0] = 0;
    CK_HIP(c, hipMemcpyAsync((void*)unprocessed, c->d_counters + 3, 4, hipMemcpyDeviceToHost, c->s_out));
    dbg_lap("enqueue parts");
    CK_HIP(c, hipStreamSynchronize(c->s_out));
    dbg_lap("sync copy-out");
    CK_HIP(c, hipStreamSynchronize(c->stream));
    dbg_lap("sync stream");
    if (idx) memcpy(idx, st_idx, n * 4);
    if (strand) memcpy(strand, st_strand, n);
    if (hash) memcpy(hash, st_hash, n * 8);
    const uint32_t lost = unprocessed[0];
    if (lost) return fail(c, CIRCKIT_ERR_TOO_LONG, "%u record(s) could not be processed", lost);
    return CIRCKIT_OK;
}

}

extern "C" {

const char* circkit_version(void) { return "circkit-mi355x 0.1.0 (gfx950)"; }

int circkit_ctx_create(int device, circkit_ctx** out)
{
    if (!out) return CIRCKIT_ERR_INVALID_ARG;
    *out = nullptr;
    int count = 0;
    if (hipGetDeviceCount(&count) != hipSuccess || count <= 0 || device < 0 || device >= count)
        return CIRCKIT_ERR_NO_DEVICE;
    circkit_ctx* c = new circkit_ctx();
    c->device = device;
    *out = c;
    CK_HIP(c, hipSetDevice(device));
    CK_HIP(c, hipStreamCreateWithFlags(&c->own_stream, hipStreamNonBlocking));
    c->stream = c->own_stream;
    CK_HIP(c, hipEventCreate(&c->ev0));
    CK_HIP(c, hipEventCreate(&c->ev1));
    CK_HIP(c, hipEventCreateWithFlags(&c->ev_order, hipEventDisableTiming));
    CK_HIP(c, hipHostMalloc((void**)&c->h_mode, 256, hipHostMallocMapped));
    c->h_mode[0] = 0; c->h_mode[1] = 0;
    CK_HIP(c, hipHostGetDevicePointer((void**)&c->d_mode, (void*)c->h_mode, 0));
    CK_HIP(c, hipMalloc(&c->d_comp, 256));
    CK_HIP(c, hipMalloc(&c->d_counters, 32 * sizeof(uint32_t)));
    CK_HIP(c, hipMemset(c->d_counters, 0, 32 * sizeof(uint32_t)));
    uint8_t comp[256];
    for (int v = 0; v < 256; ++v) comp[v] = (uint8_t)v;
    const char *x = "AGCTYRWSKMDVHBN", *y = "TCGARYWSMKHBDVN";
    for (int i = 0; x[i]; ++i) { comp[(uint8_t)x[i]] = (uint8_t)y[i]; comp[(uint8_t)x[i] + 32] = (uint8_t)(y[i] + 32); }
    CK_HIP(c, hipMemcpy(c->d_comp, comp, 256, hipMemcpyHostToDevice));
    CK_HIP(c, hipFuncSetAttribute((const void*)canon_kernel<1>, hipFuncAttributeMaxDynamicSharedMemorySize,
                                  (int)((TIER_D_DW + TIER_EXTRA_DW) * 4)));
    CK_HIP(c, hipFuncSetAttribute((const void*)canon_team_kernel, hipFuncAttributeMaxDynamicSharedMemorySize,
                                  (int)((TEAM_WAVES * TEAM_SLICE_DW + TIER_EXTRA_DW) * 4)));
    return CIRCKIT_OK;
}

int circkit_ctx_destroy(circkit_ctx* c)
{
    if (!c) return CIRCKIT_OK;
    (void)hipSetDevice(c->device);
    if (c->own_stream) (void)hipStreamSynchronize(c->own_stream);
    void* ptrs[] = { c->d_comp, c->d_counters, c->d_seg_counts, c->d_in, c->d_out, c->d_strand, c->d_off, c->d_idx, c->d_hash, c->d_table,
                     c->d_view, c->d_hashed, c->d_gscratch };
    for (void* p : ptrs) if (p) (void)hipFree(p);
    for (uint32_t* p : c->d_lists) if (p) (void)hipFree(p);
    if (c->ev0) (void)hipEventDestroy(c->ev0);
    if (c->ev1) (void)hipEventDestroy(c->ev1);
    if (c->ev_order) (void)hipEventDestroy(c->ev_order);
    if (c->ev_head) (void)hipEventDestroy(c->ev_head);
    for (hipEvent_t e : c->ev_in) if (e) (void)hipEventDestroy(e);
    for (hipEvent_t e : c->ev_done) if (e) (void)hipEventDestroy(e);
    if (c->s_in) (void)hipStreamDestroy(c->s_in);
    if (c->s_out) (void)hipStreamDestroy(c->s_out);
    if (c->h_mode) (void)hipHostFree((void*)c->h_mode);
    if (c->h_off) (void)hipHostFree((void*)c->h_off);
    if (c->orfs_release) c->orfs_release(c->orfs);
    if (c->monomerize_release) c->monomerize_release(c->monomerize);
    if (c->own_stream) (void)hipStreamDestroy(c->own_stream);
    delete c;
    return CIRCKIT_OK;
}

const char* circkit_last_error(const circkit_ctx* c) { return c ? c->err.c_str() : "null ctx"; }

static int switch_stream(circkit_ctx* c, hipStream_t s)
{
    if (s == c->stream) return CIRCKIT_OK;
    CK_HIP(c, hipSetDevice(c->device));
    if (hipEventRecord(c->ev_order, c->stream) != hipSuccess || hipStreamWaitEvent(s, c->ev_order, 0) != hipSuccess) {
        (void)hipGetLastError();
        (void)hipDeviceSynchronize();
        (void)hipGetLastError();
    }
    c->stream = s;
    return CIRCKIT_OK;
}

int circkit_ctx_set_stream(circkit_ctx* c, void* s)
{
    if (!c) return CIRCKIT_ERR_INVALID_ARG;
    return switch_stream(c, (hipStream_t)s);
}

int circkit_ctx_use_own_stream(circkit_ctx* c)
{
    if (!c) return CIRCKIT_ERR_INVALID_ARG;
    return switch_stream(c, c->own_stream);
}

int circkit_ctx_synchronize(circkit_ctx* c)
{
    if (!c) return CIRCKIT_ERR_INVALID_ARG;
    CK_HIP(c, hipSetDevice(c->device));
    CK_HIP(c, hipStreamSynchronize(c->stream));
    return CIRCKIT_OK;
}

int circkit_ctx_last_kernel_ms(circkit_ctx* c, float* ms)
{
    if (!c || !ms) return CIRCKIT_ERR_INVALID_ARG;
    if (!c->timed) return fail(c, CIRCKIT_ERR_INVALID_ARG, "no timed batch yet");
    CK_HIP(c, hipEventSynchronize(c->ev1));
    CK_HIP(c, hipEventElapsedTime(ms, c->ev0, c->ev1));
    return CIRCKIT_OK;
}

int circkit_ctx_batch_status(circkit_ctx* c, uint32_t* n_unprocessed)
{
    if (!c || !n_unprocessed) return CIRCKIT_ERR_INVALID_ARG;
    CK_HIP(c, hipSetDevice(c->device));
    *n_unprocessed = 0;
    CK_HIP(c, hipMemcpyAsync(n_unprocessed, c->d_counters + 3, 4, hipMemcpyDeviceToHost, c->stream));
    CK_HIP(c, hipStreamSynchronize(c->stream));
    if (*n_unprocessed)
        return fail(c, CIRCKIT_ERR_TOO_LONG, "%u record(s) were not processed: longer than the long-record scratch (%llu MiB, "
                    "circkit_ctx_set_long_record_scratch) or than 2^31 symbols", *n_unprocessed, (unsigned long long)(c->cap_gscratch >> 20));
    return CIRCKIT_OK;
}

int circkit_ctx_set_long_record_scratch(circkit_ctx* c, uint64_t bytes)
{
    if (!c) return CIRCKIT_ERR_INVALID_ARG;
    CK_HIP(c, hipSetDevice(c->device));
    if (bytes < (1ull << 20)) bytes = 1ull << 20;
    c->gscratch_default = bytes;
    CK_HIP(c, hipStreamSynchronize(c->stream));
    return ensure_gscratch(c, bytes);
}

int circkit_ctx_last_batch_mode(circkit_ctx* c, uint32_t* mode)
{
    if (!c || !mode) return CIRCKIT_ERR_INVALID_ARG;
    CK_HIP(c, hipSetDevice(c->device));
    CK_HIP(c, hipStreamSynchronize(c->stream));
    *mode = *c->h_mode & 3;
    return CIRCKIT_OK;
}

int circkit_canonicalize_batch_device(circkit_ctx* c, const uint8_t* d_bytes, const uint64_t* d_offsets,
                                      uint64_t n, uint8_t* d_out, uint32_t* d_idx, uint8_t* d_strand,
                                      uint64_t* d_hash)
{
    if (!c) return CIRCKIT_ERR_INVALID_ARG;
    if (n && !d_offsets) return fail(c, CIRCKIT_ERR_INVALID_ARG, "d_offsets is NULL");
    return launch_canon(c, d_bytes, d_offsets, n, d_out, d_idx, d_strand, d_hash, 0);
}

int circkit_lmsr_batch_device(circkit_ctx* c, const uint8_t* d_bytes, const uint64_t* d_offsets, uint64_t n,
                              uint8_t* d_out, uint32_t* d_idx)
{
    if (!c) return CIRCKIT_ERR_INVALID_ARG;
    if (n && !d_offsets) return fail(c, CIRCKIT_ERR_INVALID_ARG, "d_offsets is NULL");
    return launch_canon(c, d_bytes, d_offsets, n, d_out, d_idx, nullptr, nullptr, ck::CK_FLAG_FWD_ONLY);
}

int circkit_canonicalize_batch(circkit_ctx* c, const uint8_t* bytes, const uint64_t* offsets, uint64_t n,
                               uint8_t* out, uint32_t* idx, uint8_t* strand, uint64_t* hash)
{
    return host_batch(c, bytes, offsets, n, out, idx, strand, hash, 0);
}

void* circkit_host_alloc(size_t bytes)
{
    void* p = nullptr;
    return hipHostMalloc(&p, bytes ? bytes : 1, hipHostMallocDefault) == hipSuccess ? p : nullptr;
}

void circkit_host_free(void* p)
{
    if (p) (void)hipHostFree(p);
}

static int check_ascii(circkit_ctx* c, const uint8_t* s, size_t n)
{
    if (n && !s) return fail(c, CIRCKIT_ERR_INVALID_ARG, "s is NULL");
    if (n >= (1ull << 31)) return fail(c, CIRCKIT_ERR_TOO_LONG, "record too long");
    for (size_t i = 0; i < n; ++i)
        if (s[i] & 0x80) return fail(c, CIRCKIT_ERR_NOT_ASCII, "non-ASCII byte at %zu (the reference panics on non-UTF-8 / indexes by char)", i);
    return CIRCKIT_OK;
}

int circkit_lmsr_index(circkit_ctx* c, const uint8_t* s, size_t n, size_t* out_index)
{
    if (!c || !out_index) return CIRCKIT_ERR_INVALID_ARG;
    int rc = check_ascii(c, s, n);
    if (rc) return rc;
    *out_index = 0;
    if (n == 0) return CIRCKIT_OK;
    uint64_t off[2] = { 0, (uint64_t)n };
    uint32_t idx = 0;
    rc = host_batch(c, s, off, 1, nullptr, &idx, nullptr, nullptr, ck::CK_FLAG_FWD_ONLY);
    *out_index = idx;
    return rc;
}

int circkit_lmsr(circkit_ctx* c, const uint8_t* s, size_t n, uint8_t* out)
{
    if (!c || (n && !out)) return CIRCKIT_ERR_INVALID_ARG;
    int rc = check_ascii(c, s, n);
    if (rc || n == 0) return rc;
    uint64_t off[2] = { 0, (uint64_t)n };
    return host_batch(c, s, off, 1, out, nullptr, nullptr, nullptr, ck::CK_FLAG_FWD_ONLY);
}

int circkit_canonicalize(circkit_ctx* c, const uint8_t* s, size_t n, uint8_t* out)
{
    if (!c || (n && !out)) return CIRCKIT_ERR_INVALID_ARG;
    int rc = check_ascii(c, s, n);
    if (rc || n == 0) return rc;
    uint64_t off[2] = { 0, (uint64_t)n };
    return host_batch(c, s, off, 1, out, nullptr, nullptr, nullptr, 0);
}

int circkit_xxh3_64(circkit_ctx* c, const uint8_t* s, size_t n, uint64_t* out_hash)
{
    if (!c || !out_hash || (n && !s)) return CIRCKIT_ERR_INVALID_ARG;
    CK_HIP(c, hipSetDevice(c->device));
    int rc = ensure_staging(c, n, 1);
    if (rc) return rc;
    uint64_t off[2] = { 0, (uint64_t)n };
    if (n) CK_HIP(c, hipMemcpyAsync(c->d_in, s, n, hipMemcpyHostToDevice, c->stream));
    CK_HIP(c, hipMemcpyAsync(c->d_off, off, 16, hipMemcpyHostToDevice, c->stream));
    hipLaunchKernelGGL(xxh3_kernel, dim3(1), dim3(256), 0, c->stream, c->d_in, c->d_off, (uint64_t)1, c->d_hash, (const uint8_t*)nullptr, (const uint32_t*)nullptr, (const uint8_t*)nullptr);
    CK_HIP(c, hipMemcpyAsync(out_hash, c->d_hash, 8, hipMemcpyDeviceToHost, c->stream));
    CK_HIP(c, hipStreamSynchronize(c->stream));
    return CIRCKIT_OK;
}

int circkit_xxh3_batch_device(circkit_ctx* c, const uint8_t* d_bytes, const uint64_t* d_offsets, uint64_t n,
                              uint64_t* d_hash)
{
    if (!c || (n && (!d_offsets || !d_hash))) return CIRCKIT_ERR_INVALID_ARG;
    if (n == 0) return CIRCKIT_OK;
    CK_HIP(c, hipSetDevice(c->device));
    const uint64_t blocks = (n + 3) / 4;
    const unsigned grid = (unsigned)(blocks < (uint64_t)N_CU * 8 ? blocks : (uint64_t)N_CU * 8);
    hipLaunchKernelGGL(xxh3_kernel, dim3(grid), dim3(256), 0, c->stream, d_bytes, d_offsets, n, d_hash, (const uint8_t*)nullptr, (const uint32_t*)nullptr, (const uint8_t*)nullptr);
    CK_HIP(c, hipGetLastError());
    return CIRCKIT_OK;
}

#ifndef CK_UNIQ_BPC
#define CK_UNIQ_BPC 8
#endif
#ifndef CK_UNIQ_LOAD_PCT
#define CK_UNIQ_LOAD_PCT 70
#endif
static int uniq_size(circkit_ctx* c, uint64_t expected_keys)
{
    CK_HIP(c, hipSetDevice(c->device));
    uint64_t cap = 1024;
    while (cap * CK_UNIQ_LOAD_PCT < expected_keys * 100) cap <<= 1;
    if (cap - 1 != c->uniq_mask || !c->d_table) {
        c->uniq_mask = 0;
        int rc;
        if ((rc = grow(c, c->d_table, cap + 1))) return rc;
        c->uniq_mask = cap - 1;
    }
    return CIRCKIT_OK;
}
int circkit_uniq_reset(circkit_ctx* c, uint64_t expected_keys)
{
    if (!c) return CIRCKIT_ERR_INVALID_ARG;
    const int rcs = uniq_size(c, expected_keys);
    if (rcs) return rcs;
    const uint64_t cap = c->uniq_mask + 1;
    hipLaunchKernelGGL(uniq_clear_kernel, dim3(N_CU * 8), dim3(256), 0, c->stream, c->d_table, cap + 1, c->d_counters + 4);
    CK_HIP(c, hipGetLastError());
    c->uniq_count = 0;
    c->uniq_local = false;
    c->uniq_lost = false;
    return CIRCKIT_OK;
}

int circkit_uniq_first_seen(circkit_ctx* c, const uint64_t* hash, uint64_t n, uint64_t base_index, uint64_t* first_seen)
{
    if (!c || (n && (!hash || !first_seen))) return CIRCKIT_ERR_INVALID_ARG;
    if (n == 0) return CIRCKIT_OK;
    CK_HIP(c, hipSetDevice(c->device));
    if (c->uniq_lost)
        return fail(c, CIRCKIT_ERR_HIP, "the uniq table was lost in a failed rehash: the earlier batches of this stream are gone "
                    "(circkit_uniq_reset starts a new one)");
    if (c->uniq_local) { const int rc0 = circkit_uniq_reset(c, n); if (rc0) return rc0; }
    if (!c->d_table || (c->uniq_count + n) * 2 > c->uniq_mask + 1) {
        uint64_t cap = 1 << 16;
        while (cap < 4 * (c->uniq_count + n)) cap <<= 1;
        UniqSlot* nt = nullptr;
        CK_HIP(c, hipMalloc(&nt, (cap + 1) * sizeof(UniqSlot)));
        hipLaunchKernelGGL(uniq_clear_kernel, dim3(N_CU * 8), dim3(256), 0, c->stream, nt, cap + 1, (uint32_t*)nullptr);
        if (c->d_table) {
            hipLaunchKernelGGL(uniq_rehash_kernel, dim3(N_CU * 8), dim3(256), 0, c->stream, (const UniqSlot*)c->d_table, c->uniq_mask + 2, nt, cap - 1);
            hipError_t e = hipStreamSynchronize(c->stream);
            if (e == hipSuccess && getenv("CIRCKIT_TEST_FAIL_REHASH")) e = hipErrorUnknown;
            (void)hipFree(c->d_table); c->d_table = nullptr;
            if (e != hipSuccess) {
                (void)hipFree(nt);
                c->uniq_mask = 0; c->uniq_count = 0; c->uniq_lost = true;
                return fail(c, CIRCKIT_ERR_HIP, "uniq table rehash failed: %s", hipGetErrorString(e));
            }
        } else {
            CK_HIP(c, hipMemsetAsync(c->d_counters + 4, 0, 4, c->stream));
        }
        c->d_table = nt; c->uniq_mask = cap - 1;
    }
    int rc = ensure_staging(c, 0, n);
    if (rc) return rc;
    CK_HIP(c, hipMemcpyAsync(c->d_hash, hash, n * 8, hipMemcpyHostToDevice, c->stream));
    hipLaunchKernelGGL(uniq_insert_kernel, dim3(N_CU * CK_UNIQ_BPC), dim3(256), 0, c->stream, (const uint64_t*)c->d_hash, (const uint64_t*)nullptr, n, base_index,
                       c->d_table, c->uniq_mask, c->d_counters + 4);
    uint64_t* d_fs = (uint64_t*)c->d_off;
    hipLaunchKernelGGL(uniq_lookup_kernel, dim3(N_CU * CK_UNIQ_BPC), dim3(256), 0, c->stream, (const uint64_t*)c->d_hash, n, (const UniqSlot*)c->d_table,
                       c->uniq_mask, d_fs, (uint8_t*)nullptr, (uint64_t)0);
    CK_HIP(c, hipGetLastError());
    CK_HIP(c, hipMemcpyAsync(first_seen, d_fs, n * 8, hipMemcpyDeviceToHost, c->stream));
    CK_HIP(c, hipStreamSynchronize(c->stream));
    c->uniq_count += n;
    return CIRCKIT_OK;
}

int circkit_uniq_insert_device(circkit_ctx* c, const uint64_t* d_hash, uint64_t n, uint64_t base_index)
{
    if (!c || (n && !d_hash)) return CIRCKIT_ERR_INVALID_ARG;
    if (!c->d_table || c->uniq_local) return fail(c, CIRCKIT_ERR_INVALID_ARG, "circkit_uniq_reset has not been called (since the last circkit_uniq_resolve_device)");
    if (n == 0) return CIRCKIT_OK;
    CK_HIP(c, hipSetDevice(c->device));
    hipLaunchKernelGGL(uniq_insert_kernel, dim3(N_CU * CK_UNIQ_BPC), dim3(256), 0, c->stream, d_hash, (const uint64_t*)nullptr, n, base_index,
                       c->d_table, c->uniq_mask, c->d_counters + 4);
    CK_HIP(c, hipGetLastError());
    c->uniq_count += n;
    return CIRCKIT_OK;
}

int circkit_uniq_insert_pairs_device(circkit_ctx* c, const uint64_t* d_hash, const uint64_t* d_index, uint64_t n)
{
    if (!c || (n && (!d_hash || !d_index))) return CIRCKIT_ERR_INVALID_ARG;
    if (!c->d_table || c->uniq_local) return fail(c, CIRCKIT_ERR_INVALID_ARG, "circkit_uniq_reset has not been called (since the last circkit_uniq_resolve_device)");
    if (n == 0) return CIRCKIT_OK;
    CK_HIP(c, hipSetDevice(c->device));
    hipLaunchKernelGGL(uniq_insert_kernel, dim3(N_CU * CK_UNIQ_BPC), dim3(256), 0, c->stream, d_hash, d_index, n, (uint64_t)0, c->d_table,
                       c->uniq_mask, c->d_counters + 4);
    CK_HIP(c, hipGetLastError());
    c->uniq_count += n;
    return CIRCKIT_OK;
}

int circkit_uniq_lookup_device(circkit_ctx* c, const uint64_t* d_hash, uint64_t n, uint64_t* d_first_seen)
{
    if (!c || (n && (!d_hash || !d_first_seen))) return CIRCKIT_ERR_INVALID_ARG;
    if (!c->d_table || c->uniq_local) return fail(c, CIRCKIT_ERR_INVALID_ARG, "circkit_uniq_reset has not been called (since the last circkit_uniq_resolve_device)");
    if (n == 0) return CIRCKIT_OK;
    CK_HIP(c, hipSetDevice(c->device));
    hipLaunchKernelGGL(uniq_lookup_kernel, dim3(N_CU * CK_UNIQ_BPC), dim3(256), 0, c->stream, d_hash, n, (const UniqSlot*)c->d_table, c->uniq_mask, d_first_seen,
                       (uint8_t*)nullptr, (uint64_t)0);
    CK_HIP(c, hipGetLastError());
    return CIRCKIT_OK;
}

int circkit_uniq_partition_device(circkit_ctx* c, const uint64_t* d_hash, uint64_t n, uint64_t base_index, uint32_t world, uint64_t* d_rows,
                                  uint64_t* d_counts, uint32_t* d_slot)
{
    if (!c || !d_counts || world == 0 || world > UNIQ_MAX_WORLD || (n && (!d_hash || !d_rows || !d_slot))) return CIRCKIT_ERR_INVALID_ARG;
    if (n >= 0xFFFFFFFFull) return fail(c, CIRCKIT_ERR_INVALID_ARG, "circkit_uniq_partition_device: n must be < 2^32 - 1");
    if ((uintptr_t)d_rows & 15) return fail(c, CIRCKIT_ERR_INVALID_ARG, "d_rows must be 16-byte aligned");
    CK_HIP(c, hipSetDevice(c->device));
    int rc = ensure_staging(c, 0, UNIQ_MAX_WORLD);
    if (rc) return rc;
    CK_HIP(c, hipMemsetAsync(d_counts, 0, world * sizeof(uint64_t), c->stream));
    CK_HIP(c, hipMemsetAsync(c->d_hash, 0, UNIQ_MAX_WORLD * sizeof(uint64_t), c->stream));
    if (n == 0) return CIRCKIT_OK;
    hipLaunchKernelGGL(uniq_partition_count_kernel, dim3(N_CU * 8), dim3(256), 0, c->stream, d_hash, n, world, (unsigned long long*)d_counts);
    hipLaunchKernelGGL(uniq_partition_scatter_kernel, dim3(N_CU * 8), dim3(256), 0, c->stream, d_hash, n, base_index, world,
                       (const unsigned long long*)d_counts, (unsigned long long*)c->d_hash, d_rows, d_slot);
    CK_HIP(c, hipGetLastError());
    return CIRCKIT_OK;
}

int circkit_uniq_insert_rows_device(circkit_ctx* c, const uint64_t* d_rows, uint64_t n)
{
    if (!c || (n && !d_rows)) return CIRCKIT_ERR_INVALID_ARG;
    if ((uintptr_t)d_rows & 15) return fail(c, CIRCKIT_ERR_INVALID_ARG, "d_rows must be 16-byte aligned");
    if (!c->d_table || c->uniq_local) return fail(c, CIRCKIT_ERR_INVALID_ARG, "circkit_uniq_reset has not been called (since the last circkit_uniq_resolve_device)");
    if (n == 0) return CIRCKIT_OK;
    CK_HIP(c, hipSetDevice(c->device));
    hipLaunchKernelGGL(uniq_insert_rows_kernel, dim3(N_CU * CK_UNIQ_BPC), dim3(256), 0, c->stream, d_rows, n, c->d_table, c->uniq_mask, c->d_counters + 4);
    CK_HIP(c, hipGetLastError());
    c->uniq_count += n;
    return CIRCKIT_OK;
}

int circkit_uniq_lookup_rows_device(circkit_ctx* c, const uint64_t* d_rows, uint64_t n, uint64_t* d_answers)
{
    if (!c || (n && (!d_rows || !d_answers))) return CIRCKIT_ERR_INVALID_ARG;
    if ((uintptr_t)d_rows & 15) return fail(c, CIRCKIT_ERR_INVALID_ARG, "d_rows must be 16-byte aligned");
    if (!c->d_table || c->uniq_local) return fail(c, CIRCKIT_ERR_INVALID_ARG, "circkit_uniq_reset has not been called (since the last circkit_uniq_resolve_device)");
    if (n == 0) return CIRCKIT_OK;
    CK_HIP(c, hipSetDevice(c->device));
    hipLaunchKernelGGL(uniq_lookup_rows_kernel, dim3(N_CU * CK_UNIQ_BPC), dim3(256), 0, c->stream, d_rows, n, (const UniqSlot*)c->d_table, c->uniq_mask, d_answers);
    CK_HIP(c, hipGetLastError());
    return CIRCKIT_OK;
}

int circkit_uniq_gather_device(circkit_ctx* c, const uint64_t* d_answers, const uint32_t* d_slot, uint64_t n, uint64_t base_index, uint64_t* d_first_seen,
                               uint8_t* d_keep)
{
    if (!c || (n && (!d_answers || !d_slot || !d_first_seen))) return CIRCKIT_ERR_INVALID_ARG;
    if (n == 0) return CIRCKIT_OK;
    CK_HIP(c, hipSetDevice(c->device));
    hipLaunchKernelGGL(uniq_gather_kernel, dim3(N_CU * CK_UNIQ_BPC), dim3(256), 0, c->stream, d_answers, d_slot, n, base_index, d_first_seen, d_keep);
    CK_HIP(c, hipGetLastError());
    return CIRCKIT_OK;
}

int circkit_uniq_resolve_device(circkit_ctx* c, const uint64_t* d_hash, uint64_t n, uint64_t base_index, uint64_t* d_first_seen, uint8_t* d_keep)
{
    if (!c || (n && (!d_hash || !d_first_seen))) return CIRCKIT_ERR_INVALID_ARG;
    if (n >= 0xFFFFFFFFull) return fail(c, CIRCKIT_ERR_INVALID_ARG, "circkit_uniq_resolve_device: n must be < 2^32 - 1");
#ifndef CK_BKT_KEYS
#define CK_BKT_KEYS BKT_KEYS
#endif
#ifndef CK_UNIQ_BUCKET_MIN
#define CK_UNIQ_BUCKET_MIN (1u << 19)
#endif
    static const bool no_buckets = getenv("CIRCKIT_UNIQ_NO_BUCKETS") != nullptr;
    if (n >= CK_UNIQ_BUCKET_MIN && n <= ((uint64_t)CK_BKT_KEYS << BKT_MAX_LOG2) && !no_buckets) {
        int rc = uniq_size(c, n);
        if (rc) return rc;
        uint32_t log2b = 6;
        while (log2b < BKT_MAX_LOG2 && ((uint64_t)CK_BKT_KEYS << log2b) < n) ++log2b;
        const uint32_t B = 1u << log2b;
        const uint64_t per = (n + BKT_NW - 1) / BKT_NW;
        uint8_t* scratch = reinterpret_cast<uint8_t*>(c->d_table);
        uint64_t* rows = reinterpret_cast<uint64_t*>(scratch);
        uint32_t* counts = reinterpret_cast<uint32_t*>(scratch + ((n * 16 + 255) & ~255ull));
        uint32_t* tot = counts + (uint64_t)BKT_NW * B;
        uint32_t* base = tot + B;
        if ((uint64_t)(reinterpret_cast<uint8_t*>(base + B + 1) - scratch) > (c->uniq_mask + 2) * sizeof(UniqSlot))
            return fail(c, CIRCKIT_ERR_INVALID_ARG, "internal: bucket scratch does not fit the table");
        uint32_t* flag = c->d_counters + 20;
        hipLaunchKernelGGL(uniq_bkt_count_kernel, dim3(BKT_NW), dim3(1024), B * 4, c->stream, d_hash, n, per, log2b, counts, flag, c->d_counters + 4);
        hipLaunchKernelGGL(uniq_bkt_colscan_kernel, dim3(B / 64), dim3(1024), 0, c->stream, counts, B, tot);
        hipLaunchKernelGGL(uniq_bkt_basescan_kernel, dim3(1), dim3(1024), 0, c->stream, (const uint32_t*)tot, B, base);
        hipLaunchKernelGGL(uniq_bkt_scatter_kernel, dim3(BKT_NW), dim3(1024), B * 4, c->stream, d_hash, n, per, log2b, (const uint32_t*)counts, (const uint32_t*)base, rows, d_first_seen, base_index);
        hipLaunchKernelGGL(uniq_bkt_resolve_kernel, dim3(B), dim3(BKT_RESOLVE_T), 0, c->stream, (const uint64_t*)rows, (const uint32_t*)base, base_index, d_first_seen, d_keep, flag);
        if (d_keep) hipLaunchKernelGGL(uniq_keep_kernel, dim3(N_CU * CK_UNIQ_BPC), dim3(256), 0, c->stream, (const uint64_t*)d_first_seen, n, base_index, d_keep, (const uint32_t*)flag);
        hipLaunchKernelGGL(uniq_clear_kernel, dim3(N_CU * 8), dim3(256), 0, c->stream, c->d_table, c->uniq_mask + 2, (uint32_t*)nullptr, (const uint32_t*)flag);
        hipLaunchKernelGGL(uniq_resolve_insert_kernel, dim3(N_CU * CK_UNIQ_BPC), dim3(256), 0, c->stream, d_hash, n, c->d_table, c->uniq_mask, c->d_counters + 4, (const uint32_t*)flag);
        hipLaunchKernelGGL(uniq_resolve_lookup_kernel, dim3(N_CU * CK_UNIQ_BPC), dim3(256), 0, c->stream, d_hash, n, (const UniqSlot*)c->d_table, c->uniq_mask,
                           d_first_seen, d_keep, base_index, (const uint32_t*)flag);
        CK_HIP(c, hipGetLastError());
        c->uniq_local = true;
        c->uniq_count = n;
        c->uniq_lost = false;
        return CIRCKIT_OK;
    }
    int rc = circkit_uniq_reset(c, n);
    if (rc || n == 0) return rc;
    hipLaunchKernelGGL(uniq_resolve_insert_kernel, dim3(N_CU * CK_UNIQ_BPC), dim3(256), 0, c->stream, d_hash, n, c->d_table, c->uniq_mask, c->d_counters + 4);
    hipLaunchKernelGGL(uniq_resolve_lookup_kernel, dim3(N_CU * CK_UNIQ_BPC), dim3(256), 0, c->stream, d_hash, n, (const UniqSlot*)c->d_table, c->uniq_mask,
                       d_first_seen, d_keep, base_index);
    CK_HIP(c, hipGetLastError());
    c->uniq_local = true;
    c->uniq_count = n;
    return CIRCKIT_OK;
}

int circkit_uniq_status(circkit_ctx* c, uint32_t* n_overflowed)
{
    if (!c) return CIRCKIT_ERR_INVALID_ARG;
    CK_HIP(c, hipSetDevice(c->device));
    uint32_t overflow = 0;
    CK_HIP(c, hipMemcpyAsync(&overflow, c->d_counters + 4, 4, hipMemcpyDeviceToHost, c->stream));
    CK_HIP(c, hipStreamSynchronize(c->stream));
    if (n_overflowed) *n_overflowed = overflow;
    if (overflow) return fail(c, CIRCKIT_ERR_OOM, "uniq table overflow: %u key(s) found no slot (more distinct keys than circkit_uniq_reset sized it for)", overflow);
    return CIRCKIT_OK;
}

int circkit_synth_fill_device(circkit_ctx* c, uint64_t seed, uint64_t first_base, uint64_t n_bases, uint8_t* d_bytes)
{
    if (!c || (n_bases && !d_bytes)) return CIRCKIT_ERR_INVALID_ARG;
    if (n_bases == 0) return CIRCKIT_OK;
    CK_HIP(c, hipSetDevice(c->device));
    hipLaunchKernelGGL(synth_fill_kernel, dim3(N_CU * 8), dim3(256), 0, c->stream, seed, first_base, n_bases, d_bytes);
    CK_HIP(c, hipGetLastError());
    return CIRCKIT_OK;
}

int circkit_fixed_offsets_device(circkit_ctx* c, uint64_t base, uint64_t len, uint64_t n, uint64_t* d_offsets)
{
    if (!c || !d_offsets) return CIRCKIT_ERR_INVALID_ARG;
    CK_HIP(c, hipSetDevice(c->device));
    hipLaunchKernelGGL(fixed_offsets_kernel, dim3(N_CU * 4), dim3(256), 0, c->stream, base, len, n, d_offsets);
    CK_HIP(c, hipGetLastError());
    return CIRCKIT_OK;
}

int circkit_bench_copy_device(circkit_ctx* c, const void* d_src, void* d_dst, uint64_t bytes, uint32_t variant)
{
    if (!c || !d_src || !d_dst || variant >= 5) return CIRCKIT_ERR_INVALID_ARG;
    if (((uintptr_t)d_src | (uintptr_t)d_dst) & 15) return fail(c, CIRCKIT_ERR_INVALID_ARG, "circkit_bench_copy_device: 16-byte aligned buffers");
    CK_HIP(c, hipSetDevice(c->device));
    const uint64_t n16 = bytes / 16;
    const copy_v4* in = (const copy_v4*)d_src; copy_v4* out = (copy_v4*)d_dst;
    switch (variant) {
    case 0: hipLaunchKernelGGL(bench_copy_kernel<4>, dim3(2048), dim3(256), 0, c->stream, in, out, n16); break;
    case 1: hipLaunchKernelGGL(bench_copy_kernel<8>, dim3(2048), dim3(256), 0, c->stream, in, out, n16); break;
    case 2: hipLaunchKernelGGL(bench_copy_kernel<4>, dim3(8192), dim3(256), 0, c->stream, in, out, n16); break;
    case 3: hipLaunchKernelGGL(bench_copy_kernel<2>, dim3(65536), dim3(256), 0, c->stream, in, out, n16); break;
    default: CK_HIP(c, hipMemcpyAsync(d_dst, d_src, n16 * 16, hipMemcpyDeviceToDevice, c->stream)); break;
    }
    CK_HIP(c, hipGetLastError());
    return CIRCKIT_OK;
}

#ifdef CK_MIXED_TIMELINE
int circkit_debug_timeline(circkit_ctx* c, uint64_t* host, uint32_t n_wg)
{
    if (!c || !host || n_wg > 65536) return CIRCKIT_ERR_INVALID_ARG;
    CK_HIP(c, hipSetDevice(c->device));
    CK_HIP(c, hipStreamSynchronize(c->stream));
    CK_HIP(c, hipMemcpyFromSymbol(host, HIP_SYMBOL(g_timeline), (size_t)n_wg * 24));
    return CIRCKIT_OK;
}
#endif

#ifdef CK_DEBUG_POISON
int circkit_debug_poison_count(circkit_ctx* c, uint32_t* n)
{
    if (!c || !n) return CIRCKIT_ERR_INVALID_ARG;
    CK_HIP(c, hipSetDevice(c->device));
    CK_HIP(c, hipStreamSynchronize(c->stream));
    CK_HIP(c, hipMemcpy(n, c->d_counters + 12, 4, hipMemcpyDeviceToHost));
    return CIRCKIT_OK;
}
#endif

size_t circkit_normalize(const uint8_t* s, size_t n, uint8_t* out, int* changed)
{
    const uint8_t* lut = ckhost::normalize_lut();
    size_t m = 0; int ch = 0;
    for (size_t i = 0; i < n; ++i) {
        const uint8_t c = s[i], o = lut[c];
        ch |= (o != c);
        out[m] = o;
        m += (o != 0);
    }
    if (changed) *changed = ch;
    return m;
}

}
```

Baseline: 2.737 billion.

## Shorten the launch chain: fold rescue into stream kernel, run count on side stream

For the common short-sequence case the stream kernel now rescues its own deferred records in place (a MODE_FOLD flag read from the kernarg segment), so the separate rescue kernel can be skipped. The intermediate tier kernels are skipped and a direct team kernel is used. The count kernel runs on a side stream with fork/join events, and double-buffered counter sets let the counter reset happen ahead of time. The aim is fewer kernel launches and serial dependencies per batch, at the cost of more state, parity-tracked counters and extra complexity in the status path.

```diff
diff --git a/circkit_amd/csrc/circkit_hip.hip b/circkit_amd/csrc/circkit_hip.hip
--- a/circkit_amd/csrc/circkit_hip.hip
+++ b/circkit_amd/csrc/circkit_hip.hip
@@ -107,24 +107,36 @@
         }
     }
 }
-__global__ __launch_bounds__(TEAM_WAVES * 64) void canon_team_kernel(ck::CanonArgs a, uint32_t nvb, uint32_t* giants)
+template <bool DIRECT>
+__global__ __launch_bounds__(TEAM_WAVES * 64) void canon_team_kernel(ck::CanonArgs a, uint32_t nvb, uint32_t* giants, const uint32_t* mode_word, uint32_t host_mode,
+                                                                     uint32_t* mode_out, uint32_t* tiers_busy)
 {
     extern __shared__ __attribute__((aligned(16))) uint32_t lds[];
     const uint32_t total_dw = TEAM_WAVES * a.slice_dw;
     uint32_t* blk_count = lds + total_dw;
     uint32_t* lut = blk_count + 4;
     uint32_t* lutn = lut + ck::FAST_LUT_DW;
+    if (DIRECT) {
+        if (blockIdx.x == 0 && threadIdx.x == 0) *mode_out = (host_mode >> 31) ? *mode_word : host_mode & 15u;
+        if (threadIdx.x == 0) blk_count[1] = 0;
+        __syncthreads();
+    }
     {
         const uint32_t per = a.segs_per_block, mine = blockIdx.x < nvb ? (nvb - blockIdx.x + gridDim.x - 1) / gridDim.x : 0;
         uint32_t any = 0;
         for (uint32_t t = threadIdx.x; t < mine * per; t += TEAM_WAVES * 64) {
             const uint32_t sgm = (blockIdx.x + (t / per) * gridDim.x) * per + t % per;
-            if (sgm < a.in_nseg) any |= a.list_count[sgm];
+            if (sgm < a.in_nseg) {
+                const uint32_t cnt = a.list_count[sgm];
+                any |= cnt;
+                if (DIRECT && cnt) atomicAdd(blk_count + 1, cnt);
+            }
         }
         if (!__syncthreads_or((int)any)) {
             for (uint32_t t = threadIdx.x; t < mine; t += TEAM_WAVES * 64) a.defer_count[blockIdx.x + t * gridDim.x] = 0;
             return;
         }
+        if (DIRECT && threadIdx.x == 0 && blk_count[1] > mine * per) *tiers_busy = 1;
     }
     ck::fast_lut_init(lut, threadIdx.x, TEAM_WAVES * 64);
     ck::fast_lutn_init(lutn, threadIdx.x, TEAM_WAVES * 64);
@@ -132,7 +144,11 @@
     for (uint32_t vb = blockIdx.x; vb < nvb; vb += gridDim.x) {
         if (threadIdx.x == 0) *blk_count = 0;
         __syncthreads();
-        team_stage_block(a, lds, total_dw, lut, lutn, blk_count, vb, wib);
+        if (DIRECT) {
+            ck::canon_wave_loop(a, lds + wib * a.slice_dw, lut, blk_count, vb, nvb, wib, TEAM_WAVES, lutn);
+            __syncthreads();
+            ck::team_pass(a, lds, lut, lutn, blk_count, vb, wib, TEAM_WAVES, true, true);
+        } else team_stage_block(a, lds, total_dw, lut, lutn, blk_count, vb, wib);
         __syncthreads();
         if (threadIdx.x == 0) {
             a.defer_count[vb] = *blk_count;
@@ -240,11 +256,14 @@
     return (m == 2 && (al || hashed) ? 3u : m) | al | (m == 1 && !al && shortc * 2 >= n ? MODE_SHORT : 0u);
 }
 __global__ __launch_bounds__(1024) void stream_count_kernel(const uint8_t* __restrict__ bytes, const uint64_t* __restrict__ offsets, uint64_t n, uint32_t* ctl,
-                                                            uint32_t* mode, uint32_t* counters, uint32_t hashed)
+                                                            uint32_t* mode, uint32_t* own, uint32_t* next, uint32_t* ticket, uint32_t hashed)
 {
     __shared__ uint32_t blk[4];
     if (threadIdx.x < 4) blk[threadIdx.x] = 0;
-    if (blockIdx.x == 0 && threadIdx.x == 3) { counters[0] = 0; counters[1] = 0; counters[3] = 0; counters[16] = 0; counters[17] = 0; }
+    if (blockIdx.x == 0 && threadIdx.x == 3) {
+        if (own) { own[0] = 0; own[1] = 0; own[3] = 0; ticket[0] = 0; ticket[1] = 0; }
+        next[0] = 0; next[1] = 0; next[3] = 0;
+    }
     __syncthreads();
     const uint32_t shift = count_shift(n);
     const uint64_t ns = count_samples(n);
@@ -422,6 +441,43 @@
 #ifndef CK_GROUP_HASH
 #define CK_GROUP_HASH 1
 #endif
+constexpr uint32_t MODE_FOLD = 0x40000000u;
+constexpr bool stream_folds(bool hash, bool aux, bool alpha, int rows, int rpw) { return !(hash && !aux && rows == 1); }
+struct StreamKernArgs { ck::CanonArgs a; const uint32_t* mode; uint32_t host_mode, nvb; };
+typedef const __attribute__((address_space(4))) StreamKernArgs* StreamKernArgsPtr;
+static_assert(sizeof(ck::CanonArgs) % 8 == 0 && offsetof(StreamKernArgs, mode) == sizeof(ck::CanonArgs) && offsetof(StreamKernArgs, host_mode) == sizeof(ck::CanonArgs) + 8,
+              "canon_stream_kernel(CanonArgs, const uint32_t*, uint32_t, uint32_t): every argument at its natural alignment");
+__device__ __forceinline__ StreamKernArgsPtr stream_kernargs()
+{
+    StreamKernArgsPtr p = (StreamKernArgsPtr)__builtin_amdgcn_kernarg_segment_ptr();
+    asm volatile("" : "+s"(p));
+    return p;
+}
+template <bool HASH, bool AUX, bool ALPHA>
+__device__ __forceinline__ void stream_own_rescue(StreamKernArgsPtr ka, const uint32_t* lut, uint32_t* blk_count, uint32_t seg, uint32_t wpb)
+{
+    ck::CanonArgs a;
+    a.bytes = ka->a.bytes; a.offsets = ka->a.offsets; a.n_records = ka->a.n_records; a.out_bytes = ka->a.out_bytes; a.out_index = ka->a.out_index; a.out_strand = ka->a.out_strand; a.out_hash = ka->a.out_hash; a.hashed = ka->a.hashed; a.out_view = ka->a.out_view; a.list = ka->a.list; a.list_count = ka->a.list_count; a.in_nseg = ka->a.in_nseg; a.in_seg_cap = ka->a.in_seg_cap; a.segs_per_block = ka->a.segs_per_block; a.all_seg_cap = ka->a.all_seg_cap; a.taper_seg0 = ka->a.taper_seg0; a.taper_log2 = ka->a.taper_log2; a.defer_list = ka->a.defer_list; a.defer_count = ka->a.defer_count; a.out_seg_cap = ka->a.out_seg_cap; a.status = ka->a.status; a.comp_lut = ka->a.comp_lut; a.slice_dw = ka->a.slice_dw; a.flags = ka->a.flags;
+    uint32_t* const out_list = const_cast<uint32_t*>(a.list);
+    uint32_t* const out_count = const_cast<uint32_t*>(a.list_count);
+    const uint32_t left = *blk_count;
+    if (left == 0) {
+        if (threadIdx.x == 0) out_count[seg] = 0;
+        return;
+    }
+    __syncthreads();
+    if (threadIdx.x == 0) { a.defer_count[seg] = left; *blk_count = 0; }
+    __syncthreads();
+    ck::CanonArgs r = a;
+    r.list = a.defer_list; r.list_count = a.defer_count; r.in_seg_cap = a.out_seg_cap;
+    r.defer_list = out_list; r.defer_count = out_count;
+    ck::RescueState<HASH, AUX> st;
+    if (HASH) st.hc = ck::fast_hash_const();
+    ck::canon_rescue_segment<HASH, AUX, ALPHA>(r, lut, st, blk_count, seg, ck::uniform(threadIdx.x >> 6), wpb, false);
+    __syncthreads();
+    if (threadIdx.x == 0) out_count[seg] = *blk_count;
+}
+
 template <class StreamC, bool HASH, bool AUX, bool PERSIST, bool ALPHA = false>
 __global__ __launch_bounds__(StreamC::WPB * 64, (HASH && !AUX && StreamC::ROWS == 1 && (ALPHA || StreamC::RPW == 2)) ? CK_PAIR_WPE : (StreamC::WPB >= 8 || (ALPHA && !HASH && !AUX)) ? CK_FAST_WPE : 4) void canon_stream_kernel(ck::CanonArgs a, const uint32_t* __restrict__ mode,
                                                                                                              uint32_t host_mode, uint32_t nvb)
@@ -441,11 +497,16 @@
     ck::fast_lut_init(lut, threadIdx.x, StreamC::WPB * 64);
     if (GH) ck::group_hash_init(gh + 2 * StreamC::GROUP * ck::GH_STRIDE_DW, threadIdx.x);
     if (PAIR) ck::group_hash_secret_init(gh + 2 * StreamC::GROUP * ck::GH_STRIDE_DW + ck::GH_CONST_DW, threadIdx.x);
+    constexpr bool FOLDS = !PERSIST && stream_folds(HASH, AUX, ALPHA, (int)StreamC::ROWS, (int)StreamC::RPW);
     if (!PERSIST) {
         if (threadIdx.x == 0) *blk_count = 0;
         __syncthreads();
         ck::canon_stream_wave_loop<StreamC, HASH, AUX, GH, ALPHA>(a, lut, lds, blk_count, blockIdx.x, gridDim.x, gh);
         __syncthreads();
+        if (FOLDS) {
+            const StreamKernArgsPtr ka = stream_kernargs();
+            if (ka->host_mode & MODE_FOLD) { stream_own_rescue<HASH, AUX, ALPHA>(ka, lut, blk_count, blockIdx.x, StreamC::WPB); return; }
+        }
         if (threadIdx.x == 0) a.defer_count[blockIdx.x] = *blk_count;
         return;
     }
@@ -1000,6 +1061,13 @@
     UniqSlot* d_table = nullptr;
     uint64_t uniq_mask = 0, uniq_count = 0;
     uint32_t mode_seen = 0;
+    hipStream_t s_count = nullptr;
+    hipEvent_t ev_fork = nullptr, ev_join = nullptr;
+    uint32_t batch_parity = 0;
+    int clean_set = -1;
+    uint32_t* d_status = nullptr;
+    bool full_chain = false;
+    uint32_t* counter_set(uint32_t parity) const { return d_counters + 32 + 16 * (parity & 1u); }
     bool uniq_local = false;
     bool uniq_lost = false;
 
@@ -1084,6 +1152,18 @@
         if (dbg) fprintf(stderr, "[mode guess] n=%llu report=%u -> %s\n", (unsigned long long)n, seen, guess_flag ? "guessed" : "decided on the device");
     }
     const uint32_t kmode = host_mode | guess_flag;
+    const bool tiers_idle = c->h_mode[1] == 1;
+    const bool short_seq = !c->full_chain && host_mode != 0 && tiers_idle;
+    uint32_t* ctr = c->d_counters;
+    bool count_beside = false;
+    if (device_decides) {
+        ctr = c->counter_set(c->batch_parity);
+        if (short_seq && guess_flag && c->clean_set == (int)(c->batch_parity & 1u)) {
+            hipStreamCaptureStatus cap = hipStreamCaptureStatusNone;
+            count_beside = hipStreamIsCapturing(c->stream, &cap) == hipSuccess && cap == hipStreamCaptureStatusNone;
+        }
+    }
+    c->d_status = ctr + 3;
     const bool aux = d_idx || d_strand || (flags & ck::CK_FLAG_FWD_ONLY);
     const uint64_t per_step = aux ? StreamCAux::GROUP : StreamC::GROUP;
     const uint64_t blocks = (n + per_step - 1) / per_step;
@@ -1131,16 +1211,28 @@
     ck::CanonArgs a{};
     a.bytes = d_bytes; a.offsets = d_offsets; a.n_records = n;
     a.out_bytes = d_out; a.out_index = d_idx; a.out_strand = d_strand; a.out_hash = d_hash; a.hashed = c->d_hashed; a.out_view = view;
-    a.comp_lut = c->d_comp; a.status = c->d_counters + 3; a.flags = flags;
+    a.comp_lut = c->d_comp; a.status = ctr + 3; a.flags = flags;
     a.list = nullptr; a.list_count = nullptr; a.all_seg_cap = all_cap; a.taper_seg0 = taper_seg0; a.taper_log2 = taper_log2;
     a.defer_list = c->d_lists[0]; a.defer_count = c->d_seg_counts; a.out_seg_cap = cap;
     a.slice_dw = 0;
     const uint32_t* counts = c->d_counters + 5;
+    const bool fold_ok = short_seq && (host_mode & 3) != 3;
+    if (fold_ok) { a.list = c->d_lists[1]; a.list_count = c->d_seg_counts + c->seg_alloc; }
+    bool folded = false;
     {
         if (device_decides) {
             const uint64_t ns = count_samples(n);
             const unsigned cgrid = (unsigned)((ns + 1023) / 1024 < 128 ? (ns + 1023) / 1024 : 128);
-            hipLaunchKernelGGL(stream_count_kernel, dim3(cgrid), dim3(1024), 0, c->stream, d_bytes, d_offsets, n, c->d_counters + 8, c->d_counters + 5, c->d_counters, (d_hash && !aux) ? 1u : 0u);
+            uint32_t* next = c->counter_set(c->batch_parity + 1);
+            if (count_beside) {
+                CK_HIP(c, hipEventRecord(c->ev_fork, c->stream));
+                CK_HIP(c, hipStreamWaitEvent(c->s_count, c->ev_fork, 0));
+            }
+            hipLaunchKernelGGL(stream_count_kernel, dim3(cgrid), dim3(1024), 0, count_beside ? c->s_count : c->stream, d_bytes, d_offsets, n, c->d_counters + 8,
+                               c->d_counters + 5, count_beside ? (uint32_t*)nullptr : ctr, next, c->d_counters + 16, (d_hash && !aux) ? 1u : 0u);
+            if (count_beside) CK_HIP(c, hipEventRecord(c->ev_join, c->s_count));
+            c->batch_parity ^= 1u;
+            c->clean_set = (int)(c->batch_parity & 1u);
         }
         const uint32_t seen = *c->h_mode;
         const uint32_t expect = host_mode ? host_mode & 3 : ((seen & 3) ? seen & 3 : 1u);
@@ -1155,8 +1247,10 @@
                 const dim3 grid(full ? G : small);
 #define CK_LAUNCH_STREAM(CFG, H, A, BLK, AL)                                                                                         \
                 do {                                                                                                                \
-                    if (full) hipLaunchKernelGGL((canon_stream_kernel<CFG, H, A, false, AL>), grid, BLK, 0, c->stream, a, counts, kmode, G); \
-                    else hipLaunchKernelGGL((canon_stream_kernel<CFG, H, A, true, AL>), grid, BLK, 0, c->stream, a, counts, kmode, G);       \
+                    const uint32_t km = kmode | (fold_ok && full && stream_folds(H, A, AL, (int)CFG::ROWS, (int)CFG::RPW) ? MODE_FOLD : 0u);    \
+                    folded = (km & MODE_FOLD) != 0;                                                                                 \
+                    if (full) hipLaunchKernelGGL((canon_stream_kernel<CFG, H, A, false, AL>), grid, BLK, 0, c->stream, a, counts, km, G); \
+                    else hipLaunchKernelGGL((canon_stream_kernel<CFG, H, A, true, AL>), grid, BLK, 0, c->stream, a, counts, km, G);       \
                 } while (0)
                 if (rows == 1) {
                     if (aux) CK_LAUNCH_STREAM(StreamCAux, true, true, block_aux, false);
@@ -1168,10 +1262,13 @@
                             if (host_mode && (sh != 0) != expect_short) continue;
                             const bool full_sh = full && (sh != 0) == expect_short;
                             const dim3 grid_sh(full_sh ? G : small);
-                            if (sh) { if (full_sh) hipLaunchKernelGGL((canon_stream_kernel<StreamCHP, false, false, false, false>), grid_sh, block_hp, 0, c->stream, a, counts, kmode, G);
-                                      else hipLaunchKernelGGL((canon_stream_kernel<StreamCHP, false, false, true, false>), grid_sh, block_hp, 0, c->stream, a, counts, kmode, G); }
-                            else { if (full_sh) hipLaunchKernelGGL((canon_stream_kernel<StreamC, false, false, false, false>), grid_sh, block, 0, c->stream, a, counts, kmode, G);
-                                   else hipLaunchKernelGGL((canon_stream_kernel<StreamC, false, false, true, false>), grid_sh, block, 0, c->stream, a, counts, kmode, G); }
+                            static_assert(stream_folds(false, false, false, 1, 1) && stream_folds(false, false, false, 1, 2), "the bytes-only builds carry the own-segment rescue");
+                            const uint32_t km = kmode | (fold_ok && full_sh ? MODE_FOLD : 0u);
+                            folded = fold_ok && full_sh;
+                            if (sh) { if (full_sh) hipLaunchKernelGGL((canon_stream_kernel<StreamCHP, false, false, false, false>), grid_sh, block_hp, 0, c->stream, a, counts, km, G);
+                                      else hipLaunchKernelGGL((canon_stream_kernel<StreamCHP, false, false, true, false>), grid_sh, block_hp, 0, c->stream, a, counts, km, G); }
+                            else { if (full_sh) hipLaunchKernelGGL((canon_stream_kernel<StreamC, false, false, false, false>), grid_sh, block, 0, c->stream, a, counts, km, G);
+                                   else hipLaunchKernelGGL((canon_stream_kernel<StreamC, false, false, true, false>), grid_sh, block, 0, c->stream, a, counts, km, G); }
                         }
                     }
                 } else {
@@ -1195,15 +1292,17 @@
 #else
         uint32_t* mode_out = c->d_mode;
 #endif
-        const bool mixed_has_it = host_mode && !aux && (host_mode & 3) == 3;
+        if (short_seq) mode_out = c->d_counters + 6;
+        const uint32_t rmode = short_seq ? host_mode : kmode;
+        const bool mixed_has_it = (host_mode && !aux && (host_mode & 3) == 3) || folded;
         const bool lean = (!host_mode || !(host_mode & MODE_ALPHA)) && !mixed_has_it, alpha = (!host_mode || (host_mode & MODE_ALPHA)) && !mixed_has_it;
-        if (aux) hipLaunchKernelGGL((canon_rescue_kernel<true, true, false>), dim3(grid), dim3(256), 0, c->stream, a, counts, kmode, mode_out, c->d_counters + 1);
+        if (aux) { if (!folded) hipLaunchKernelGGL((canon_rescue_kernel<true, true, false>), dim3(grid), dim3(256), 0, c->stream, a, counts, rmode, mode_out, ctr + 1); }
         else if (d_hash) {
-            if (lean) hipLaunchKernelGGL((canon_rescue_kernel<true, false, false>), dim3(grid), dim3(256), 0, c->stream, a, counts, kmode, mode_out, c->d_counters + 1);
-            if (alpha) hipLaunchKernelGGL((canon_rescue_kernel<true, false, true>), dim3(grid), dim3(256), 0, c->stream, a, counts, kmode, mode_out, c->d_counters + 1);
+            if (lean) hipLaunchKernelGGL((canon_rescue_kernel<true, false, false>), dim3(grid), dim3(256), 0, c->stream, a, counts, rmode, mode_out, ctr + 1);
+            if (alpha) hipLaunchKernelGGL((canon_rescue_kernel<true, false, true>), dim3(grid), dim3(256), 0, c->stream, a, counts, rmode, mode_out, ctr + 1);
         } else {
-            if (lean) hipLaunchKernelGGL((canon_rescue_kernel<false, false, false>), dim3(grid), dim3(256), 0, c->stream, a, counts, kmode, mode_out, c->d_counters + 1);
-            if (alpha) hipLaunchKernelGGL((canon_rescue_kernel<false, false, true>), dim3(grid), dim3(256), 0, c->stream, a, counts, kmode, mode_out, c->d_counters + 1);
+            if (lean) hipLaunchKernelGGL((canon_rescue_kernel<false, false, false>), dim3(grid), dim3(256), 0, c->stream, a, counts, rmode, mode_out, ctr + 1);
+            if (alpha) hipLaunchKernelGGL((canon_rescue_kernel<false, false, true>), dim3(grid), dim3(256), 0, c->stream, a, counts, rmode, mode_out, ctr + 1);
         }
     }
     if (!aux && (!host_mode || (host_mode & 3) == 3)) {
@@ -1214,6 +1313,8 @@
 #else
         uint32_t* mode_out = c->d_mode;
 #endif
+        if (short_seq) mode_out = c->d_counters + 6;
+        const uint32_t mmode = short_seq ? host_mode : kmode;
         for (uint32_t nm = 0; nm < 2; ++nm) {
             if (host_mode && ((host_mode & MODE_ALPHA) != 0) != (nm != 0)) continue;
             const bool expected = host_mode ? true : ((seen & 3) == 3 && ((seen & MODE_ALPHA) != 0) == (nm != 0));
@@ -1233,11 +1334,11 @@
             const int mwpb = nm ? mixed_wpb(true, d_hash != nullptr) : (d_hash ? mixed_wpb(false, true) : mixed_wpb(false, false));
             const size_t shmem = ((size_t)mwpb * a.slice_dw + 4 + ck::FAST_LUT_DW + ck::LEAN_LUTN_DW + (d_hash ? ck::LEAN_HASH_TABLE_DW : 0)) * 4;
             if (d_hash) {
-                if (nm) hipLaunchKernelGGL(canon_mixed_nh_kernel, dim3(grid), dim3(64 * mwpb), shmem, c->stream, a, counts, kmode, mode_out, c->d_counters + 1, ticket);
-                else hipLaunchKernelGGL(canon_mixed_h_kernel, dim3(grid), dim3(64 * mwpb), shmem, c->stream, a, counts, kmode, mode_out, c->d_counters + 1, ticket);
+                if (nm) hipLaunchKernelGGL(canon_mixed_nh_kernel, dim3(grid), dim3(64 * mwpb), shmem, c->stream, a, counts, mmode, mode_out, ctr + 1, ticket);
+                else hipLaunchKernelGGL(canon_mixed_h_kernel, dim3(grid), dim3(64 * mwpb), shmem, c->stream, a, counts, mmode, mode_out, ctr + 1, ticket);
             } else {
-                if (nm) hipLaunchKernelGGL(canon_mixed_n_kernel, dim3(grid), dim3(64 * mwpb), shmem, c->stream, a, counts, kmode, mode_out, c->d_counters + 1, ticket);
-                else hipLaunchKernelGGL(canon_mixed_kernel, dim3(grid), dim3(64 * mwpb), shmem, c->stream, a, counts, kmode, mode_out, c->d_counters + 1, ticket);
+                if (nm) hipLaunchKernelGGL(canon_mixed_n_kernel, dim3(grid), dim3(64 * mwpb), shmem, c->stream, a, counts, mmode, mode_out, ctr + 1, ticket);
+                else hipLaunchKernelGGL(canon_mixed_kernel, dim3(grid), dim3(64 * mwpb), shmem, c->stream, a, counts, mmode, mode_out, ctr + 1, ticket);
             }
         }
     }
@@ -1272,12 +1373,13 @@
         fprintf(stderr, "[dump] stage A input: %llu records in %u segments\n", (unsigned long long)total, nseg);
     }
 #endif
-    const bool tiers_idle = c->h_mode[1] == 1;
     for (int t = 0; t < BATCH_TIERS; ++t) {
         const bool last = t == BATCH_TIERS - 1;
+        if (short_seq && !last) continue;
+        const int in = short_seq ? 1 : t + 1;
         const unsigned spb = t == 0 ? 1 : (last ? (nseg + N_CU - 1) / N_CU : (nseg >= 16u * N_CU ? 4 : 1));
         const unsigned grid = (nseg + spb - 1) / spb;
-        a.list = c->d_lists[t + 1]; a.list_count = c->d_seg_counts + (uint64_t)(t + 1) * c->seg_alloc;
+        a.list = c->d_lists[in]; a.list_count = c->d_seg_counts + (uint64_t)in * c->seg_alloc;
         a.in_nseg = nseg; a.in_seg_cap = seg_cap; a.segs_per_block = spb;
         a.defer_list = last ? c->d_lists[0] : c->d_lists[t + 2];
         a.defer_count = last ? c->d_seg_counts : c->d_seg_counts + (uint64_t)(t + 2) * c->seg_alloc;
@@ -1285,7 +1387,12 @@
         a.slice_dw = last ? TEAM_SLICE_DW : BATCH_SLICE_DW[t];
         const unsigned bpc = tiers_idle ? CK_TIER_BPC_IDLE : CK_TIER_BPC;
         const unsigned launched = grid < (unsigned)N_CU * bpc ? grid : (unsigned)N_CU * bpc;
-        if (last) hipLaunchKernelGGL(canon_team_kernel, dim3(launched), dim3(TEAM_WAVES * 64), (TEAM_WAVES * TEAM_SLICE_DW + TIER_EXTRA_DW) * 4, c->stream, a, grid, c->d_counters);
+        if (last && short_seq) {
+            if (count_beside) CK_HIP(c, hipStreamWaitEvent(c->stream, c->ev_join, 0));
+            hipLaunchKernelGGL(canon_team_kernel<true>, dim3(launched), dim3(TEAM_WAVES * 64), (TEAM_WAVES * TEAM_SLICE_DW + TIER_EXTRA_DW) * 4, c->stream, a, grid, ctr,
+                               counts, kmode, c->d_mode, ctr + 1);
+        } else if (last) hipLaunchKernelGGL(canon_team_kernel<false>, dim3(launched), dim3(TEAM_WAVES * 64), (TEAM_WAVES * TEAM_SLICE_DW + TIER_EXTRA_DW) * 4, c->stream, a, grid, ctr,
+                                            (const uint32_t*)nullptr, 0u, (uint32_t*)nullptr, (uint32_t*)nullptr);
         else if (tiers_idle) hipLaunchKernelGGL((canon_kernel<4, false>), dim3(launched), dim3(256), (4 * a.slice_dw + TIER_EXTRA_DW) * 4, c->stream, a, grid, (uint32_t*)nullptr);
         else hipLaunchKernelGGL((canon_kernel<4, true>), dim3(launched), dim3(256), (4 * a.slice_dw + TIER_EXTRA_DW) * 4, c->stream, a, grid, (uint32_t*)nullptr);
         nseg = grid;
@@ -1305,8 +1412,8 @@
         a2.in_nseg = w1; a2.in_seg_cap = spb1 * seg_cap; a2.segs_per_block = w1;
         a2.defer_list = nullptr; a2.defer_count = nullptr; a2.out_seg_cap = 0;
         a2.slice_dw = (uint32_t)(cap_dw < 0xFFFFFFFFull ? cap_dw : 0xFFFFFFFFull);
-        hipLaunchKernelGGL(canon_global_kernel, dim3(w1), dim3(TEAM_WAVES * 64), 0, c->stream, a, a2, c->d_gscratch, c->d_counters + 2, (const uint32_t*)c->d_counters,
-                           (const uint32_t*)(c->d_counters + 1), c->d_mode + 1);
+        hipLaunchKernelGGL(canon_global_kernel, dim3(w1), dim3(TEAM_WAVES * 64), 0, c->stream, a, a2, c->d_gscratch, c->d_counters + 2, (const uint32_t*)ctr,
+                           (const uint32_t*)(ctr + 1), c->d_mode + 1);
     }
     if (d_hash) {
         if (view) hipLaunchKernelGGL(xxh3_kernel, dim3(G < 2048u ? G : 2048u), dim3(256), 0, c->stream, d_bytes, d_offsets, n, d_hash, (const uint8_t*)c->d_hashed,
@@ -1328,6 +1435,7 @@
     a.out_bytes = d_out; a.out_index = d_idx; a.out_strand = d_strand; a.out_hash = nullptr; a.hashed = nullptr;
     a.comp_lut = c->d_comp; a.status = c->d_counters + 3; a.flags = flags;
     CK_HIP(c, hipMemsetAsync(c->d_counters + 3, 0, sizeof(uint32_t), c->stream));
+    c->d_status = c->d_counters + 3;
     const uint64_t need = worst_case_dw(len);
     int t = 0;
     while (t < N_TIERS && TIER_DW[t] < need) ++t;
@@ -1431,7 +1539,7 @@
         if (strand) CK_HIP(c, hipMemcpyAsync(strand, c->d_strand, n, hipMemcpyDeviceToHost, c->stream));
         if (hash) CK_HIP(c, hipMemcpyAsync(hash, c->d_hash, n * 8, hipMemcpyDeviceToHost, c->stream));
         uint32_t unprocessed = 0;
-        CK_HIP(c, hipMemcpyAsync(&unprocessed, c->d_counters + 3, 4, hipMemcpyDeviceToHost, c->stream));
+        CK_HIP(c, hipMemcpyAsync(&unprocessed, c->d_status, 4, hipMemcpyDeviceToHost, c->stream));
         CK_HIP(c, hipStreamSynchronize(c->stream));
         if (unprocessed) return fail(c, CIRCKIT_ERR_TOO_LONG, "%u record(s) could not be processed", unprocessed);
         return CIRCKIT_OK;
@@ -1521,7 +1629,7 @@
         if (hash) CK_HIP(c, hipMemcpyAsync(st_hash + r0, c->d_hash + r0, nk * 8, hipMemcpyDeviceToHost, c->s_out));
     }
     unprocessed[0] = 0;
-    CK_HIP(c, hipMemcpyAsync((void*)unprocessed, c->d_counters + 3, 4, hipMemcpyDeviceToHost, c->s_out));
+    CK_HIP(c, hipMemcpyAsync((void*)unprocessed, c->d_status, 4, hipMemcpyDeviceToHost, c->s_out));
     dbg_lap("enqueue parts");
     CK_HIP(c, hipStreamSynchronize(c->s_out));
     dbg_lap("sync copy-out");
@@ -1561,8 +1669,13 @@
     c->h_mode[0] = 0; c->h_mode[1] = 0;
     CK_HIP(c, hipHostGetDevicePointer((void**)&c->d_mode, (void*)c->h_mode, 0));
     CK_HIP(c, hipMalloc(&c->d_comp, 256));
-    CK_HIP(c, hipMalloc(&c->d_counters, 32 * sizeof(uint32_t)));
-    CK_HIP(c, hipMemset(c->d_counters, 0, 32 * sizeof(uint32_t)));
+    CK_HIP(c, hipMalloc(&c->d_counters, 64 * sizeof(uint32_t)));
+    CK_HIP(c, hipMemset(c->d_counters, 0, 64 * sizeof(uint32_t)));
+    c->d_status = c->d_counters + 3;
+    c->full_chain = getenv("CIRCKIT_FULL_CHAIN") != nullptr;
+    CK_HIP(c, hipStreamCreateWithFlags(&c->s_count, hipStreamNonBlocking));
+    CK_HIP(c, hipEventCreateWithFlags(&c->ev_fork, hipEventDisableTiming));
+    CK_HIP(c, hipEventCreateWithFlags(&c->ev_join, hipEventDisableTiming));
     uint8_t comp[256];
     for (int v = 0; v < 256; ++v) comp[v] = (uint8_t)v;
     const char *x = "AGCTYRWSKMDVHBN", *y = "TCGARYWSMKHBDVN";
@@ -1570,7 +1683,9 @@
     CK_HIP(c, hipMemcpy(c->d_comp, comp, 256, hipMemcpyHostToDevice));
     CK_HIP(c, hipFuncSetAttribute((const void*)canon_kernel<1>, hipFuncAttributeMaxDynamicSharedMemorySize,
                                   (int)((TIER_D_DW + TIER_EXTRA_DW) * 4)));
-    CK_HIP(c, hipFuncSetAttribute((const void*)canon_team_kernel, hipFuncAttributeMaxDynamicSharedMemorySize,
+    CK_HIP(c, hipFuncSetAttribute((const void*)canon_team_kernel<false>, hipFuncAttributeMaxDynamicSharedMemorySize,
+                                  (int)((TEAM_WAVES * TEAM_SLICE_DW + TIER_EXTRA_DW) * 4)));
+    CK_HIP(c, hipFuncSetAttribute((const void*)canon_team_kernel<true>, hipFuncAttributeMaxDynamicSharedMemorySize,
                                   (int)((TEAM_WAVES * TEAM_SLICE_DW + TIER_EXTRA_DW) * 4)));
     return CIRCKIT_OK;
 }
@@ -1580,6 +1695,9 @@
     if (!c) return CIRCKIT_OK;
     (void)hipSetDevice(c->device);
     if (c->own_stream) (void)hipStreamSynchronize(c->own_stream);
+    if (c->s_count) { (void)hipStreamSynchronize(c->s_count); (void)hipStreamDestroy(c->s_count); }
+    if (c->ev_fork) (void)hipEventDestroy(c->ev_fork);
+    if (c->ev_join) (void)hipEventDestroy(c->ev_join);
     void* ptrs[] = { c->d_comp, c->d_counters, c->d_seg_counts, c->d_in, c->d_out, c->d_strand, c->d_off, c->d_idx, c->d_hash, c->d_table,
                      c->d_view, c->d_hashed, c->d_gscratch };
     for (void* p : ptrs) if (p) (void)hipFree(p);
@@ -1650,7 +1768,7 @@
     if (!c || !n_unprocessed) return CIRCKIT_ERR_INVALID_ARG;
     CK_HIP(c, hipSetDevice(c->device));
     *n_unprocessed = 0;
-    CK_HIP(c, hipMemcpyAsync(n_unprocessed, c->d_counters + 3, 4, hipMemcpyDeviceToHost, c->stream));
+    CK_HIP(c, hipMemcpyAsync(n_unprocessed, c->d_status, 4, hipMemcpyDeviceToHost, c->stream));
     CK_HIP(c, hipStreamSynchronize(c->stream));
     if (*n_unprocessed)
         return fail(c, CIRCKIT_ERR_TOO_LONG, "%u record(s) were not processed: longer than the long-record scratch (%llu MiB, "
@@ -2070,7 +2188,9 @@
     if (!c || !n) return CIRCKIT_ERR_INVALID_ARG;
     CK_HIP(c, hipSetDevice(c->device));
     CK_HIP(c, hipStreamSynchronize(c->stream));
-    CK_HIP(c, hipMemcpy(n, c->d_counters + 12, 4, hipMemcpyDeviceToHost));
+    uint32_t all[64];
+    CK_HIP(c, hipMemcpy(all, c->d_counters, sizeof all, hipMemcpyDeviceToHost));
+    *n = all[12] + all[32 + 12] + all[48 + 12];
     return CIRCKIT_OK;
 }
 #endif
```

Measured after the change: 2.673 billion. -2.4%, worse.
